# HKUST-Aerial-Robotics/MIND

Hardware: AMD Instinct MI355X
Metric: sim steps/sec (whole node) + scenario-tree nodes expanded/sec, AV2 demo scenes (higher is better)
Workload: dtype f32-class (bf16 hi+mid+lo split operands = 24 significand bits, six products, fp32 accumulate) pair kernel + ActorNet, f32 elsewhere in the predictor, f64 iLQR

## Files before the change

### include/mind_hip.h

```cpp
#ifndef MIND_HIP_H
#define MIND_HIP_H

#include <stddef.h>
#include <stdint.h>

#ifdef __cplusplus
extern "C" {
#endif

#define MIND_OK 0
#define MIND_EINVAL (-1)
#define MIND_ENOMEM (-2)
#define MIND_EHIP (-3)
#define MIND_ESTATE (-4)
#define MIND_ENOTFOUND (-5)

typedef struct mind_ctx mind_ctx;

int mind_ctx_create(int device, void *stream, mind_ctx **out);
int mind_ctx_destroy(mind_ctx *ctx);
const char *mind_last_error_string(mind_ctx *ctx);
int mind_ctx_synchronize(mind_ctx *ctx);

typedef struct {
  const char *name;
  const float *data;
  int64_t numel;
} mind_tensor_desc;

int mind_weights_load(mind_ctx *ctx, const mind_tensor_desc *tensors, int n_tensors);

typedef struct {
  int n_scenes;
  const int32_t *actor_off;
  const int32_t *lane_off;
  const float *actors;
  const float *lanes;
  const float *lane_feat;
  const float *actor_ctrs;
  const float *actor_vecs;
  const float *lane_ctrs;
  const float *lane_vecs;
  const float *const *rpe;
  const float *tgt_nodes;
  const float *tgt_rpe;
} mind_scene_batch;

typedef struct {
  float *cls;
  float *reg;
  float *vel;
  float *lane_feat;
  float *actor_emb;
  float *cls_emb;
} mind_pred_out;

int mind_predict_batch(mind_ctx *ctx, const mind_scene_batch *in, mind_pred_out *out);

typedef struct {
  float *cov_vel;
  float *param;
} mind_pred_aux;
int mind_predict_batch_aux(mind_ctx *ctx, const mind_scene_batch *in, mind_pred_out *out, const mind_pred_aux *aux);

#define MIND_BASIS_BEZIER 0
#define MIND_BASIS_MONOMIAL 1
int mind_set_decoder_basis(mind_ctx *ctx, int basis);
int mind_get_decoder_basis(mind_ctx *ctx);

#define MIND_CURVE_MAX_POINTS (1LL << 26)
int mind_curve_eval(mind_ctx *ctx, int basis, const float *param, long long n_rows, const double *tau, int n_tau,
                    float *reg, float *vel, float *cov_vel);
int mind_debug_curve_basis(int basis, const double *tau, int n_tau, float *T, float *Tp);

int mind_last_fusion_stats(mind_ctx *ctx, int *n_launches, float *total_ms, double *pairs_processed);
int mind_last_actor_stats(mind_ctx *ctx, int *layerwise, int *n_launches, int *n_chunks, float *total_ms);
int mind_last_token_stats(mind_ctx *ctx, int *layerwise, int *n_launches, int *n_chunks, float *total_ms);
int mind_last_token_stage_ms(mind_ctx *ctx, float *out_ms, int cap);
int mind_last_ilqr_stats(mind_ctx *ctx, float *kernel_ms, int *n_trees, int *workgroups_per_tree);
int mind_last_ilqr_profile(mind_ctx *ctx, double *out9);
int mind_last_ilqr_trace(mind_ctx *ctx, int tree, int phase, double *out, int cap_rows, int *n_rows);
int mind_set_profiling(mind_ctx *ctx, int enable);

#define MIND_PAIR_F32 0
#define MIND_PAIR_BF16X3 1
#define MIND_PAIR_BF16 2
#define MIND_PAIR_BF16X6 3
int mind_set_pair_precision(mind_ctx *ctx, int mode);

int mind_set_tuning(mind_ctx *ctx, const char *name, int value);
int mind_get_pair_precision(mind_ctx *ctx);
int mind_debug_pack_bfrag(const float *w, int row_stride, uint32_t *out);

int mind_debug_pair_schedule(const int *scene_tokens, const int *scene_actors, int n_scenes, int n_cu, int last_layer, int *out_jobs, int cap,
                             int *out_info);

int mind_debug_predict_choice(const char *const *knob_names, const int *knob_values, int n_knobs, int pair_prec, int n_cu, int have_side,
                              const int *scene_actors, const int *scene_lanes, int n_scenes, long long *out, int cap);

int mind_debug_ilqr_plan(const char *const *knob_names, const int *knob_values, int n_knobs, int n_cu, int mode, int n_trees, const int *n_nodes,
                         const int32_t *parents, long long *out, int cap, int *bad);

int mind_debug_aime_book(int pred_len, int max_depth, int max_rounds, int n_agents, int world, int rank, int force, int n_rounds, const int *dec_len,
                         const float *dec, int n_tokens, int bytes_per_pair, int plan_chunk_mb, int per_scene, long long *out, int cap, char *msg,
                         int msg_cap);

int mind_debug_wait_word(const unsigned *word, unsigned want, double timeout_s, double (*clock)(void *user), void *user, int spins_per_look);

int mind_debug_actor_lw_plan(int n_actors, int np, int chunk, long long *out_launches, int cap, long long *out_info);

int mind_debug_token_lw_plan(int n_tokens, int mode, int chunk, long long *out_launches, int cap, long long *out_info);

int mind_debug_pack_conv_frag(const float *w, int co, int ci, int ksz, uint32_t *out, size_t cap);

int mind_debug_pack(const char *what, const float *w, int a, int b, int c, float *out, size_t cap);
int mind_debug_weight_image(const mind_tensor_desc *tensors, int n_tensors, float *blob, size_t blob_cap, char *names, size_t names_cap,
                            long long *entries, int entries_cap, long long *out_info, char *msg, int msg_cap);
int mind_debug_weight_bind(const mind_tensor_desc *tensors, int n_tensors, const char *drop, char *msg, int msg_cap);

int mind_debug_trig(mind_ctx *ctx, const double *x, int n, double *out);

int mind_debug_set_layers(mind_ctx *ctx, int n);
int64_t mind_debug_read(mind_ctx *ctx, const char *name, float *host, int64_t max_floats);

typedef struct {
  int n_nodes;
  const int32_t *parent;
  const float *prob;
  int n_agents;
  const float *agent_mean;
  const float *agent_cov;
  const double *field;
  const double *node_w;
} mind_cost_tree;

typedef struct {
  double dt, wheelbase;
  double w_des_state[6];
  double w_state_con[6];
  double state_lower[6], state_upper[6];
  double w_ctrl[2];
  double w_tgt, w_ego, w_ego_cov_offset, w_exo, w_exo_cov_offset, w_exo_cost_offset;
  double grid_res; int grid_w, grid_h;
  int max_iter;
} mind_ilqr_cfg;

typedef struct { int iterations; int converged; double J; double mu; } mind_ilqr_stats;

int mind_ilqr_solve_trees(mind_ctx *ctx, const mind_ilqr_cfg *cfg, const mind_cost_tree *trees,
                          int n_trees, const double *x0, const double *target_lane, int n_lane_pts,
                          double target_vel, int use_exo, const double *us_init, double *xs,
                          double *us, mind_ilqr_stats *stats);

int mind_ilqr_contingency(mind_ctx *ctx, const mind_ilqr_cfg *cfg_warm, const mind_ilqr_cfg *cfg_full,
                          const mind_cost_tree *trees, int n_trees, const double *x0,
                          const double *target_lane, int n_lane_pts, double target_vel, double *xs,
                          double *us, mind_ilqr_stats *stats_warm, mind_ilqr_stats *stats_full);
int mind_ilqr_contingency_begin(mind_ctx *ctx, const mind_ilqr_cfg *cfg_warm, const mind_ilqr_cfg *cfg_full,
                                const mind_cost_tree *trees, int n_trees, const double *x0,
                                const double *target_lane, int n_lane_pts, double target_vel, double *xs,
                                double *us, mind_ilqr_stats *stats_warm, mind_ilqr_stats *stats_full);
int mind_ilqr_contingency_begin_plan(mind_ctx *ctx, const mind_ilqr_cfg *cfg_warm, const mind_ilqr_cfg *cfg_full, const double *x0,
                                     const double *target_lane, int n_lane_pts, double target_vel, double *xs, double *us,
// ... 334 lines not shown
```

### mind_amd/_lib.py

```python
import ctypes as C
import os

_HERE = os.path.dirname(os.path.abspath(__file__))
LIB_PATH = os.environ.get("MIND_HIP_LIB", os.path.join(_HERE, "libmind_hip.so"))

WAIT_CLOCK = C.CFUNCTYPE(C.c_double, C.c_void_p)
MIND_OK = 0
MIND_EINVAL, MIND_ENOMEM, MIND_EHIP, MIND_ESTATE, MIND_ENOTFOUND = -1, -2, -3, -4, -5


class TensorDesc(C.Structure):
    _fields_ = [("name", C.c_char_p), ("data", C.POINTER(C.c_float)), ("numel", C.c_int64)]


class SceneBatch(C.Structure):
    _fields_ = [("n_scenes", C.c_int), ("actor_off", C.POINTER(C.c_int32)), ("lane_off", C.POINTER(C.c_int32)),
                ("actors", C.c_void_p), ("lanes", C.c_void_p), ("lane_feat", C.c_void_p),
                ("actor_ctrs", C.c_void_p), ("actor_vecs", C.c_void_p), ("lane_ctrs", C.c_void_p),
                ("lane_vecs", C.c_void_p), ("rpe", C.POINTER(C.c_void_p)), ("tgt_nodes", C.c_void_p),
                ("tgt_rpe", C.c_void_p)]


class PredOut(C.Structure):
    _fields_ = [("cls", C.c_void_p), ("reg", C.c_void_p), ("vel", C.c_void_p), ("lane_feat", C.c_void_p),
# ... 108 lines not shown

class AimeNode(C.Structure):
    _fields_ = [("round", C.c_int), ("scene", C.c_int), ("mode", C.c_int), ("parent", C.c_int), ("prob", C.c_float),
                ("cur_t", C.c_int), ("end_t", C.c_int), ("flags", C.c_int), ("dur", C.c_int), ("row_off", C.c_int64),
                ("tgt_pts", C.c_float * 22)]


class AimePlanOut(C.Structure):
    _fields_ = [("nodes", C.POINTER(AimeNode)), ("n_nodes", C.c_int), ("rows", C.POINTER(C.c_float)), ("n_row_floats", C.c_int64),
                ("n_expanded", C.c_int), ("n_rounds", C.c_int), ("root_flags", C.c_int), ("round_scenes", C.c_int * 32),
                ("pair_ms", C.c_float), ("pair_launches", C.c_int), ("n_trees", C.c_int), ("tree_top", C.POINTER(C.c_int32)),
                ("tree_off", C.POINTER(C.c_int32)), ("flat_parent", C.POINTER(C.c_int32)), ("flat_prob", C.POINTER(C.c_float)),
                ("flat_mean", C.POINTER(C.c_float)), ("flat_cov", C.POINTER(C.c_float)), ("solves_begun", C.c_int)]


class IlqrCfg(C.Structure):
    _fields_ = [("dt", C.c_double), ("wheelbase", C.c_double), ("w_des_state", C.c_double * 6),
                ("w_state_con", C.c_double * 6), ("state_lower", C.c_double * 6), ("state_upper", C.c_double * 6),
                ("w_ctrl", C.c_double * 2), ("w_tgt", C.c_double), ("w_ego", C.c_double),
                ("w_ego_cov_offset", C.c_double), ("w_exo", C.c_double), ("w_exo_cov_offset", C.c_double),
                ("w_exo_cost_offset", C.c_double), ("grid_res", C.c_double), ("grid_w", C.c_int), ("grid_h", C.c_int),
                ("max_iter", C.c_int)]


class IlqrStats(C.Structure):
    _fields_ = [("iterations", C.c_int), ("converged", C.c_int), ("J", C.c_double), ("mu", C.c_double)]


LOOP_TAN_FN = C.CFUNCTYPE(C.c_double, C.c_double)
LOOP_SINCOS_FN = C.CFUNCTYPE(None, C.c_double, C.POINTER(C.c_double))


class LoopDesc(C.Structure):
    _fields_ = [("n_tracks", C.c_int), ("n_steps", C.c_int), ("clamp_last", C.c_int), ("ego_state", C.c_void_p), ("ego_state_is_f32", C.c_int), ("ego_obs", C.c_void_p), ("ego_trig32", C.c_void_p),
                ("tan_fn", C.c_void_p), ("sincos_fn", C.c_void_p), ("exo_obs", C.c_void_p),
                ("exo_valid", C.c_void_p), ("timestep", C.c_void_p), ("type_slot", C.c_void_p),
                ("sim_step", C.c_double), ("plan_step", C.c_double), ("enable_time", C.c_double),
                ("wheelbase", C.c_double), ("max_speed", C.c_double), ("max_steer", C.c_double), ("max_acc", C.c_double), ("max_dec", C.c_double),
                ("n_lanes", C.c_int), ("lane_pts", C.c_void_p), ("lane_flags", C.c_void_p),
                ("n_lane_pts", C.c_int), ("target_lane", C.c_void_p), ("target_lane_info", C.c_void_p),
                ("time_ahead", C.c_double), ("min_vel", C.c_float), ("dist_thres", C.c_float), ("max_depth", C.c_int), ("max_rounds", C.c_int),
                ("pred_len", C.c_int), ("prob_floor", C.c_float),
                ("cfg_warm", C.c_void_p), ("cfg_full", C.c_void_p), ("solve_n_lane_pts", C.c_int), ("solve_lane", C.c_void_p), ("target_vel", C.c_double),
                ("eval_n_lane_pts", C.c_int), ("eval_lane_is_f32", C.c_int), ("eval_lane", C.c_void_p), ("speculative", C.c_int)]


class LoopTotals(C.Structure):
    _fields_ = [("plans", C.c_longlong), ("expansions", C.c_longlong), ("scen_trees", C.c_longlong), ("rounds", C.c_longlong),
                ("aime_s", C.c_double), ("ilqr_s", C.c_double), ("total_s", C.c_double),
                ("iterations", C.c_longlong), ("node_iterations", C.c_longlong), ("node_iterations_exo", C.c_longlong),
                ("warm_speculated", C.c_longlong), ("warm_hits", C.c_longlong),
                ("pair_ms", C.c_double), ("pair_launches", C.c_longlong), ("scene_n2", C.c_double), ("scene_n_a1", C.c_double),
                ("ilqr_ms", C.c_double), ("ilqr_launches", C.c_longlong), ("ilqr_trees", C.c_longlong), ("ilqr_workgroups_per_tree", C.c_int),
                ("ilqr_prof", C.c_double * 9), ("ilqr_node_steps", C.c_double)]


class LoopOut(C.Structure):
    _fields_ = [("planned", C.c_int), ("enabled", C.c_int), ("n_steps", C.c_longlong), ("n_plans", C.c_longlong), ("episode_steps", C.c_longlong),
                ("sim_time", C.c_double), ("last_trigger", C.c_double), ("state", C.c_double * 4), ("ctrl", C.c_double * 2),
                ("n_agents", C.c_int), ("n_trees", C.c_int), ("best", C.c_int), ("n_expanded", C.c_int), ("n_rounds", C.c_int), ("n_traj_nodes", C.c_int),
                ("costs", C.POINTER(C.c_double)), ("aime_s", C.c_double), ("ilqr_s", C.c_double), ("total_s", C.c_double),
                ("tot", LoopTotals)]


PLANNER_EGO_KEY = -(1 << 63)


class PlannerDesc(C.Structure):
    _fields_ = [("time_ahead", C.c_double), ("min_vel", C.c_float), ("dist_thres", C.c_float), ("max_depth", C.c_int), ("max_rounds", C.c_int),
                ("pred_len", C.c_int), ("prob_floor", C.c_float), ("cfg_warm", C.c_void_p), ("cfg_full", C.c_void_p), ("speculative", C.c_int),
                ("ego_type_slot", C.c_int)]


class PlannerOut(C.Structure):
    _fields_ = [("n_plans", C.c_longlong),
                ("n_agents", C.c_int), ("n_trees", C.c_int), ("best", C.c_int), ("n_expanded", C.c_int), ("n_rounds", C.c_int), ("n_traj_nodes", C.c_int),
                ("costs", C.POINTER(C.c_double)), ("ctrl", C.c_double * 2), ("aime_s", C.c_double), ("ilqr_s", C.c_double), ("total_s", C.c_double),
                ("tot", LoopTotals)]


EXPORTS = ["mind_ctx_create", "mind_ctx_destroy", "mind_last_error_string", "mind_ctx_synchronize",
           "mind_weights_load", "mind_predict_batch", "mind_last_fusion_stats", "mind_last_actor_stats", "mind_debug_actor_lw_plan", "mind_last_token_stats", "mind_last_token_stage_ms", "mind_debug_token_lw_plan", "mind_set_profiling",
           "mind_ilqr_solve_trees", "mind_ilqr_contingency", "mind_ilqr_solve_fields", "mind_cost_eval", "mind_ilqr_score_trees", "mind_ilqr_gains", "mind_ilqr_policy_rollouts", "mind_lane_dist_field", "mind_aime_world", "mind_aime_rebase", "mind_debug_aime_decide", "mind_debug_set_layers",
           "mind_debug_read", "mind_set_pair_precision", "mind_get_pair_precision", "mind_debug_pack_bfrag", "mind_debug_pack_conv_frag", "mind_debug_pack", "mind_debug_weight_image", "mind_debug_weight_bind", "mind_debug_pair_schedule", "mind_debug_predict_choice", "mind_debug_ilqr_plan", "mind_debug_aime_book", "mind_set_tuning", "mind_last_ilqr_stats", "mind_aime_plan", "mind_last_ilqr_profile", "mind_eval_traj_trees", "mind_last_ilqr_trace", "mind_ilqr_contingency_begin", "mind_ilqr_finish", "mind_fill_tracks", "mind_ilqr_contingency_begin_plan", "mind_debug_trig", "mind_aime_plan_begin", "mind_aime_plan_poll", "mind_aime_plan_finish", "mind_ctx_busy", "mind_ilqr_finish_plan",
           "mind_set_exchange", "mind_last_exchange_stats", "mind_debug_wait_word",
           "mind_predict_batch_aux", "mind_set_decoder_basis", "mind_get_decoder_basis", "mind_curve_eval", "mind_debug_curve_basis",
           "mind_audit_plan", "mind_audit_episode", "mind_debug_box_clearance",
           "mind_forecast_score", "mind_debug_forecast_score",
           "mind_audit_road_plan", "mind_audit_road_episode", "mind_debug_road_margin",
           "mind_loop_create", "mind_loop_destroy", "mind_loop_reset", "mind_loop_advance", "mind_loop_state", "mind_loop_last_plan", "mind_loop_export",
           "mind_planner_create", "mind_planner_destroy", "mind_planner_reset", "mind_planner_observe", "mind_planner_set_lanes", "mind_planner_set_target_lane",
           "mind_planner_set_solve_lane", "mind_planner_set_eval_lane", "mind_planner_plan", "mind_planner_last_plan", "mind_planner_export"]

EXCHANGE_FN = C.CFUNCTYPE(C.c_int, C.c_void_p, C.c_int, C.c_void_p, C.c_void_p, C.c_int64)
XCHG_ALLGATHER, XCHG_ALLREDUCE, XCHG_ALLTOALLV = 0, 1, 2

_lib = None


def load():
    global _lib
    if _lib is not None:
        return _lib
    if not os.path.exists(LIB_PATH):
        raise ImportError(f"{LIB_PATH} is missing: the HIP extension must be built (hipcc --offload-arch=gfx950); "
                          "there is no CPU fallback for the product path")
    lib = C.CDLL(LIB_PATH)
    lib.mind_ctx_create.argtypes = [C.c_int, C.c_void_p, C.POINTER(C.c_void_p)]
    lib.mind_ctx_destroy.argtypes = [C.c_void_p]
    lib.mind_last_error_string.argtypes = [C.c_void_p]
    lib.mind_last_error_string.restype = C.c_char_p
    lib.mind_ctx_synchronize.argtypes = [C.c_void_p]
    lib.mind_weights_load.argtypes = [C.c_void_p, C.POINTER(TensorDesc), C.c_int]
    lib.mind_predict_batch.argtypes = [C.c_void_p, C.POINTER(SceneBatch), C.POINTER(PredOut)]
    lib.mind_predict_batch_aux.argtypes = [C.c_void_p, C.POINTER(SceneBatch), C.POINTER(PredOut), C.POINTER(PredAux)]
    lib.mind_set_decoder_basis.argtypes = [C.c_void_p, C.c_int]
    lib.mind_get_decoder_basis.argtypes = [C.c_void_p]
    lib.mind_curve_eval.argtypes = [C.c_void_p, C.c_int, C.c_void_p, C.c_longlong, C.POINTER(C.c_double), C.c_int, C.c_void_p, C.c_void_p, C.c_void_p]
    lib.mind_debug_curve_basis.argtypes = [C.c_int, C.POINTER(C.c_double), C.c_int, C.POINTER(C.c_float), C.POINTER(C.c_float)]
    lib.mind_last_fusion_stats.argtypes = [C.c_void_p, C.POINTER(C.c_int), C.POINTER(C.c_float), C.POINTER(C.c_double)]
    lib.mind_last_actor_stats.argtypes = [C.c_void_p, C.POINTER(C.c_int), C.POINTER(C.c_int), C.POINTER(C.c_int), C.POINTER(C.c_float)]
    lib.mind_debug_actor_lw_plan.argtypes = [C.c_int, C.c_int, C.c_int, C.POINTER(C.c_longlong), C.c_int, C.POINTER(C.c_longlong)]
    lib.mind_last_token_stats.argtypes = [C.c_void_p, C.POINTER(C.c_int), C.POINTER(C.c_int), C.POINTER(C.c_int), C.POINTER(C.c_float)]
    lib.mind_last_token_stage_ms.argtypes = [C.c_void_p, C.POINTER(C.c_float), C.c_int]
    lib.mind_debug_token_lw_plan.argtypes = [C.c_int, C.c_int, C.c_int, C.POINTER(C.c_longlong), C.c_int, C.POINTER(C.c_longlong)]
    lib.mind_set_profiling.argtypes = [C.c_void_p, C.c_int]
    lib.mind_ilqr_solve_trees.argtypes = [C.c_void_p, C.POINTER(IlqrCfg), C.POINTER(CostTree), C.c_int,
                                          C.POINTER(C.c_double), C.POINTER(C.c_double), C.c_int, C.c_double, C.c_int,
                                          C.POINTER(C.c_double), C.POINTER(C.c_double), C.POINTER(C.c_double),
                                          C.POINTER(IlqrStats)]
    lib.mind_ilqr_contingency.argtypes = [C.c_void_p, C.POINTER(IlqrCfg), C.POINTER(IlqrCfg), C.POINTER(CostTree), C.c_int,
                                          C.POINTER(C.c_double), C.POINTER(C.c_double), C.c_int, C.c_double,
                                          C.POINTER(C.c_double), C.POINTER(C.c_double), C.POINTER(IlqrStats), C.POINTER(IlqrStats)]
    lib.mind_ilqr_contingency_begin.argtypes = [C.c_void_p, C.POINTER(IlqrCfg), C.POINTER(IlqrCfg), C.POINTER(CostTree), C.c_int,
                                          C.POINTER(C.c_double), C.POINTER(C.c_double), C.c_int, C.c_double,
                                          C.POINTER(C.c_double), C.POINTER(C.c_double), C.POINTER(IlqrStats), C.POINTER(IlqrStats)]
    lib.mind_ilqr_finish.argtypes = [C.c_void_p]
    lib.mind_ilqr_contingency_begin_plan.argtypes = [C.c_void_p, C.POINTER(IlqrCfg), C.POINTER(IlqrCfg), C.c_void_p, C.c_void_p, C.c_int, C.c_double,
                                                     C.c_void_p, C.c_void_p, C.c_void_p, C.c_void_p]
    lib.mind_fill_tracks.argtypes = [C.c_void_p, C.c_int, C.c_int, C.c_void_p, C.c_void_p, C.c_void_p, C.c_void_p, C.c_void_p, C.c_void_p]
    lib.mind_ilqr_solve_fields.argtypes = [C.c_void_p, C.POINTER(IlqrCfg), C.POINTER(FieldGrid), C.POINTER(CostTree), C.c_int,
                                           C.POINTER(C.c_double), C.POINTER(C.c_double), C.POINTER(C.c_double),
                                           C.POINTER(C.c_double), C.POINTER(IlqrStats)]
    lib.mind_cost_eval.argtypes = [C.c_void_p, C.POINTER(IlqrCfg), C.POINTER(FieldGrid), C.POINTER(CostTree),
                                   C.POINTER(C.c_double), C.POINTER(C.c_double), C.c_int, C.c_double, C.c_int, C.c_int,
                                   C.POINTER(C.c_int32), C.POINTER(C.c_double), C.POINTER(C.c_double), C.POINTER(C.c_double)]
    lib.mind_ilqr_score_trees.argtypes = [C.c_void_p, C.POINTER(IlqrCfg), C.POINTER(FieldGrid), C.POINTER(CostTree), C.c_int,
                                          C.POINTER(C.c_double), C.POINTER(C.c_double), C.c_int, C.c_double, C.c_int, C.c_int,
                                          C.POINTER(C.c_double), C.POINTER(C.c_double), C.POINTER(C.c_double), C.POINTER(C.c_double)]
    lib.mind_ilqr_gains.argtypes = [C.c_void_p, C.POINTER(IlqrCfg), C.POINTER(FieldGrid), C.POINTER(CostTree), C.c_int,
                                    C.POINTER(C.c_double), C.POINTER(C.c_double), C.c_int, C.c_double, C.c_int,
                                    C.POINTER(C.c_double), C.POINTER(C.c_double), C.POINTER(IlqrGainsOut)]
    lib.mind_ilqr_policy_rollouts.argtypes = [C.c_void_p, C.POINTER(IlqrCfg), C.POINTER(FieldGrid), C.POINTER(CostTree), C.c_int,
                                              C.POINTER(C.c_double), C.POINTER(C.c_double), C.c_int, C.c_double, C.c_int,
                                              C.POINTER(C.c_double), C.POINTER(C.c_double), C.POINTER(C.c_double), C.c_int,
                                              C.POINTER(C.c_double), C.POINTER(C.c_double), C.POINTER(C.c_double), C.POINTER(C.c_double),
                                              C.POINTER(C.c_double), C.POINTER(C.c_double)]
    lib.mind_lane_dist_field.argtypes = [C.c_void_p, C.POINTER(C.c_double), C.POINTER(C.c_double), C.c_int, C.c_int, C.c_int,
                                         C.c_double] + [C.POINTER(C.c_double)] * 4
    lib.mind_aime_world.argtypes = [C.c_void_p, C.POINTER(WorldIn), C.POINTER(WorldOut)]
    lib.mind_aime_rebase.argtypes = [C.c_void_p, C.POINTER(RebaseIn), C.POINTER(RebaseOut)]
    lib.mind_debug_aime_decide.argtypes = [C.c_void_p, C.c_int, C.POINTER(C.c_int32), C.POINTER(C.c_int32), C.c_void_p, C.POINTER(C.c_float), C.c_void_p,
                                           C.c_void_p, C.c_void_p, C.c_int, C.c_float, C.c_float, C.c_int, C.c_int, C.c_void_p, C.c_void_p, C.c_void_p]
    lib.mind_aime_plan.argtypes = [C.c_void_p, C.POINTER(AimePlanIn), C.POINTER(AimePlanOut)]
    lib.mind_aime_plan_begin.argtypes = [C.c_void_p, C.POINTER(AimePlanIn)]
    lib.mind_aime_plan_poll.argtypes = [C.c_void_p]
    lib.mind_aime_plan_finish.argtypes = [C.c_void_p, C.POINTER(AimePlanOut)]
    lib.mind_ctx_busy.argtypes = [C.c_void_p]
    lib.mind_ilqr_finish_plan.argtypes = [C.c_void_p, C.c_int, C.c_int, C.c_void_p, C.c_void_p, C.c_void_p, C.c_void_p]
    lib.mind_set_pair_precision.argtypes = [C.c_void_p, C.c_int]
    lib.mind_set_tuning.argtypes = [C.c_void_p, C.c_char_p, C.c_int]
    lib.mind_last_ilqr_stats.argtypes = [C.c_void_p, C.POINTER(C.c_float), C.POINTER(C.c_int), C.POINTER(C.c_int)]
    lib.mind_last_ilqr_profile.argtypes = [C.c_void_p, C.POINTER(C.c_double)]
    lib.mind_last_ilqr_trace.argtypes = [C.c_void_p, C.c_int, C.c_int, C.POINTER(C.c_double), C.c_int, C.POINTER(C.c_int)]
    lib.mind_eval_traj_trees.argtypes = [C.POINTER(C.c_double), C.POINTER(C.c_double), C.POINTER(C.c_int32), C.c_int, C.c_void_p, C.c_int, C.c_int,
                                         C.c_double, C.POINTER(C.c_double)]
    lib.mind_get_pair_precision.argtypes = [C.c_void_p]
    lib.mind_debug_pack_bfrag.argtypes = [C.POINTER(C.c_float), C.c_int, C.POINTER(C.c_uint32)]
    lib.mind_debug_pair_schedule.argtypes = [C.POINTER(C.c_int), C.POINTER(C.c_int), C.c_int, C.c_int, C.c_int, C.POINTER(C.c_int), C.c_int, C.POINTER(C.c_int)]
    lib.mind_debug_predict_choice.argtypes = [C.POINTER(C.c_char_p), C.POINTER(C.c_int), C.c_int, C.c_int, C.c_int, C.c_int, C.POINTER(C.c_int), C.POINTER(C.c_int),
                                              C.c_int, C.POINTER(C.c_longlong), C.c_int]
    lib.mind_debug_ilqr_plan.argtypes = [C.POINTER(C.c_char_p), C.POINTER(C.c_int), C.c_int, C.c_int, C.c_int, C.c_int, C.POINTER(C.c_int), C.POINTER(C.c_int32),
                                         C.POINTER(C.c_longlong), C.c_int, C.POINTER(C.c_int)]
    lib.mind_debug_wait_word.argtypes = [C.POINTER(C.c_uint), C.c_uint, C.c_double, WAIT_CLOCK, C.c_void_p, C.c_int]
    lib.mind_debug_aime_book.argtypes = [C.c_int] * 8 + [C.POINTER(C.c_int), C.POINTER(C.c_float)] + [C.c_int] * 4 + [C.POINTER(C.c_longlong), C.c_int, C.c_char_p, C.c_int]
    lib.mind_debug_trig.argtypes = [C.c_void_p, C.POINTER(C.c_double), C.c_int, C.POINTER(C.c_double)]
    lib.mind_debug_pack_conv_frag.argtypes = [C.POINTER(C.c_float), C.c_int, C.c_int, C.c_int, C.POINTER(C.c_uint32), C.c_size_t]
    lib.mind_debug_pack.argtypes = [C.c_char_p, C.POINTER(C.c_float), C.c_int, C.c_int, C.c_int, C.POINTER(C.c_float), C.c_size_t]
    lib.mind_debug_weight_image.argtypes = [C.POINTER(TensorDesc), C.c_int, C.POINTER(C.c_float), C.c_size_t, C.c_char_p, C.c_size_t,
                                            C.POINTER(C.c_longlong), C.c_int, C.POINTER(C.c_longlong), C.c_char_p, C.c_int]
    lib.mind_debug_weight_bind.argtypes = [C.POINTER(TensorDesc), C.c_int, C.c_char_p, C.c_char_p, C.c_int]
    lib.mind_debug_set_layers.argtypes = [C.c_void_p, C.c_int]
    lib.mind_debug_read.argtypes = [C.c_void_p, C.c_char_p, C.POINTER(C.c_float), C.c_int64]
    lib.mind_set_exchange.argtypes = [C.c_void_p, C.c_int, C.c_int, EXCHANGE_FN, C.c_void_p, C.c_int]
    lib.mind_last_exchange_stats.argtypes = [C.c_void_p, C.POINTER(C.c_longlong), C.POINTER(C.c_longlong)]
    lib.mind_loop_create.argtypes = [C.c_void_p, C.POINTER(LoopDesc), C.POINTER(C.c_void_p)]
    lib.mind_loop_destroy.argtypes = [C.c_void_p]
    lib.mind_loop_reset.argtypes = [C.c_void_p]
    lib.mind_loop_advance.argtypes = [C.c_void_p, C.c_int, C.c_double, C.c_longlong, C.POINTER(LoopOut)]
    lib.mind_loop_state.argtypes = [C.c_void_p, C.POINTER(LoopOut)]
    lib.mind_loop_last_plan.argtypes = [C.c_void_p, C.POINTER(AimePlanOut)] + [C.POINTER(C.c_void_p)] * 6 + [C.c_void_p]
    lib.mind_loop_export.argtypes = [C.c_void_p, C.c_int, C.POINTER(C.c_int), C.c_void_p, C.c_void_p, C.c_void_p]
    lib.mind_planner_create.argtypes = [C.c_void_p, C.POINTER(PlannerDesc), C.POINTER(C.c_void_p)]
    lib.mind_planner_destroy.argtypes = [C.c_void_p]
    lib.mind_planner_reset.argtypes = [C.c_void_p]
    lib.mind_planner_observe.argtypes = [C.c_void_p, C.c_int, C.c_void_p, C.c_int, C.c_void_p, C.c_void_p, C.c_void_p]
    lib.mind_planner_set_lanes.argtypes = [C.c_void_p, C.c_int, C.c_void_p, C.c_void_p]
    lib.mind_planner_set_target_lane.argtypes = [C.c_void_p, C.c_int, C.c_void_p, C.c_void_p]
    lib.mind_planner_set_solve_lane.argtypes = [C.c_void_p, C.c_int, C.c_void_p, C.c_double]
    lib.mind_planner_set_eval_lane.argtypes = [C.c_void_p, C.c_int, C.c_void_p, C.c_int]
    lib.mind_planner_plan.argtypes = [C.c_void_p, C.c_void_p, C.c_void_p, C.POINTER(PlannerOut)]
    lib.mind_planner_last_plan.argtypes = [C.c_void_p, C.POINTER(AimePlanOut)] + [C.POINTER(C.c_void_p)] * 6 + [C.c_void_p]
    lib.mind_planner_export.argtypes = [C.c_void_p, C.c_int, C.POINTER(C.c_int), C.c_void_p, C.c_void_p, C.c_void_p]
    lib.mind_audit_plan.argtypes = [C.c_void_p, C.POINTER(AuditBox), C.c_double, C.POINTER(CostTree), C.c_int, C.c_int, C.POINTER(C.c_double),
                                    C.POINTER(AuditPlanOut)]
    lib.mind_audit_episode.argtypes = [C.c_void_p, C.POINTER(AuditBox), C.c_int, C.c_int, C.c_int, C.POINTER(C.c_double), C.POINTER(C.c_double),
                                       C.POINTER(C.c_uint8), C.POINTER(C.c_double), C.POINTER(AuditEpisodeOut)]
    lib.mind_debug_box_clearance.argtypes = [C.c_int, C.c_int, C.POINTER(C.c_double), C.POINTER(C.c_double), C.POINTER(C.c_double), C.POINTER(C.c_double)]
    fc_tail = [C.POINTER(ForecastCfg), C.c_int, C.POINTER(C.c_int32), C.c_void_p, C.c_void_p, C.POINTER(C.c_double), C.POINTER(C.c_uint8),
               C.POINTER(C.c_uint8), C.POINTER(ForecastOut)]
    lib.mind_forecast_score.argtypes = [C.c_void_p] + fc_tail
    lib.mind_debug_forecast_score.argtypes = fc_tail
    road = [C.POINTER(C.c_double), C.POINTER(C.c_int32), C.c_int]
    lib.mind_audit_road_plan.argtypes = [C.c_void_p, C.POINTER(AuditBox)] + road + [C.POINTER(CostTree), C.c_int, C.c_int, C.POINTER(C.c_double),
                                                                                   C.POINTER(AuditRoadPlanOut)]
    lib.mind_audit_road_episode.argtypes = [C.c_void_p, C.POINTER(AuditBox)] + road + [C.c_int, C.c_int, C.POINTER(C.c_double),
                                                                                      C.POINTER(AuditRoadEpisodeOut)]
    lib.mind_debug_road_margin.argtypes = [C.c_int, C.POINTER(C.c_double), C.POINTER(AuditBox)] + road + [C.POINTER(C.c_double), C.POINTER(C.c_double)] + \
        [C.POINTER(C.c_int32)] * 3
    for n in EXPORTS:
        getattr(lib, n)
        if n not in ("mind_last_error_string", "mind_debug_read"):
            getattr(lib, n).restype = C.c_int
    lib.mind_debug_read.restype = C.c_int64
    _lib = lib
    return lib


PRED_CHOICE_FIELDS = ("header", "n_runs", "np", "actor_form", "actor_arg", "actor_grid", "actor_chunk", "actor_chunks", "actor_launches", "qsplit", "qk_stride",
                      "tiled", "edge_bf16", "edge_pair_bytes", "tok_chunk", "tok_lw", "tok_chunks", "pair_family", "pair_np", "l5_jobs5", "xcd_lanes",
                      "xcd_lanes5", "dec_actor", "dec_np", "fp32_dec", "split_dec", "want_mw", "mw_blocks", "cls_on_side", "tgt_wait_first",
                      "dec_head_ra")
PAIR_PREC = ("f32", "bf16x3", "bf16", "bf16x6")


def predict_choice(knobs, prec, scenes, n_cu=256, have_side=True):
    lib = load()
    names = (C.c_char_p * max(1, len(knobs)))(*[k.encode() for k in knobs])
    vals = (C.c_int * max(1, len(knobs)))(*[int(v) for v in knobs.values()])
    sa = (C.c_int * len(scenes))(*[a for a, _ in scenes])
    sl = (C.c_int * len(scenes))(*[l for _, l in scenes])
    cap = 32 + 6 * len(scenes)
    out = (C.c_longlong * cap)()
    n = lib.mind_debug_predict_choice(names, vals, len(knobs), PAIR_PREC.index(prec) if isinstance(prec, str) else prec, n_cu, int(have_side),
                                      sa, sl, len(scenes), out, cap)
    if n == MIND_EINVAL:
# ... 256 lines not shown
```

### mind_amd/csrc/aime_plan.hip

```cpp
#include <chrono>
namespace {

int pl_pin(mind_ctx *c, int which, size_t bytes) {
  if (bytes <= c->pl_pin_cap[which]) return MIND_OK;
  if (c->pl_pin[which]) (void)hipHostFree(c->pl_pin[which]);
  c->pl_pin[which] = nullptr; c->pl_pin_cap[which] = 0;
  const size_t want = bytes < ((size_t)64 << 20) ? std::max<size_t>(2 * bytes, (size_t)1 << 20) : bytes + bytes / 2 + 4096;
  if (hipHostMalloc(&c->pl_pin[which], want, hipHostMallocDefault) != hipSuccess)
    return fail(c, MIND_ENOMEM, "hipHostMalloc(%zu) failed", want);
  c->pl_pin_cap[which] = want;
  return MIND_OK;
}

struct CopySeg { const float *src; float *dst; long long n; };
__global__ __launch_bounds__(256) void k_copy_segs(const CopySeg *__restrict__ segs) {
  const CopySeg S = segs[blockIdx.y];
  const long long i0 = (long long)blockIdx.x * 2048 + threadIdx.x;
#pragma unroll
  for (int k = 0; k < 8; ++k) {
    const long long i = i0 + k * 256;
    if (i < S.n) S.dst[i] = S.src[i];
  }
}

int pl_exchange(mind_ctx *c, int op, void *send, void *recv, size_t bytes) {
  HIPCHK(c, hipStreamSynchronize(c->stream));
  const int rc = c->xfn(c->xuser, op, send, recv, (int64_t)bytes);
  if (rc) return fail(c, MIND_EHIP, "mind_aime_plan: the exchange callback failed (%d)", rc);
  c->x_collectives += 1;
  c->x_bytes += op == MIND_XCHG_ALLGATHER ? (long long)bytes * c->xw : (long long)bytes;
  return MIND_OK;
}

int pl_exchange_v(mind_ctx *c, void *send, void *recv, const int64_t *table) {
  HIPCHK(c, hipStreamSynchronize(c->stream));
  const int rc = c->xfn(c->xuser, MIND_XCHG_ALLTOALLV, send, recv, (int64_t)(intptr_t)table);
  if (rc) return fail(c, MIND_EHIP, "mind_aime_plan: the exchange callback failed (%d)", rc);
  c->x_collectives += 1;
  for (int r = 0; r < c->xw; ++r) c->x_bytes += (long long)table[(size_t)c->xw + r];
  return MIND_OK;
}

int pl_copy_segs(mind_ctx *c, const std::vector<CopySeg> &segs) {
  if (segs.empty()) return MIND_OK;
  long long mx = 0;
  for (const CopySeg &s : segs) mx = std::max(mx, s.n);
  if (mx == 0) return MIND_OK;
  int rc;
  if ((rc = ensure(c, c->x_seg, segs.size() * sizeof(CopySeg)))) return rc;
  if ((rc = pl_pin(c, 6, segs.size() * sizeof(CopySeg)))) return rc;
  memcpy(c->pl_pin[6], segs.data(), segs.size() * sizeof(CopySeg));
  HIPCHK(c, hipMemcpyAsync(c->x_seg.p, c->pl_pin[6], segs.size() * sizeof(CopySeg), hipMemcpyHostToDevice, c->stream));
  hipLaunchKernelGGL(k_copy_segs, dim3((unsigned)((mx + 2047) / 2048), (unsigned)segs.size()), dim3(256), 0, c->stream, (const CopySeg *)c->x_seg.p);
  HIPCHK(c, hipGetLastError());
  return MIND_OK;
}

static_assert(PL_K == AIME_K && PL_OBS == RB_T, "aime_book.h restates the kernels' constants");
static_assert(sizeof(PlJob) == sizeof(AimeGather) && sizeof(PlJob) == sizeof(AimeFlat) && offsetof(PlJob, row0) == offsetof(AimeGather, row0) &&
                  offsetof(PlJob, row0) == offsetof(AimeFlat, row0) && offsetof(PlJob, n) == offsetof(AimeGather, dur) && offsetof(PlJob, n) == offsetof(AimeFlat, n) &&
                  offsetof(PlJob, dst) == offsetof(AimeGather, dst) && offsetof(PlJob, dst) == offsetof(AimeFlat, dst) && offsetof(PlJob, a) == offsetof(AimeGather, a) &&
                  offsetof(PlJob, a) == offsetof(AimeFlat, a), "JobTable holds the packing kernels' job records");

struct PlTrace {
  std::chrono::steady_clock::time_point t0 = std::chrono::steady_clock::now();
  void operator()(const char *what) const {
    static const bool on = getenv("MIND_PLAN_TRACE") != nullptr;
    if (on) fprintf(stderr, "[plan] %8.1f us  %s\n", std::chrono::duration<double, std::micro>(std::chrono::steady_clock::now() - t0).count(), what);
  }
};

double pl_steady_now(void *) { return std::chrono::duration<double>(std::chrono::steady_clock::now().time_since_epoch()).count(); }

struct PlanRun {
  mind_ctx *c;
  const mind_aime_plan_in *in;
  mind_aime_plan_out *out;
  hipStream_t st;
  AimeBook &book;
  const int a, l, P, HZ;
  const bool raw;
  const int XW, XR;
  const bool dist;
  const RootLayout ro;
  const float *droot = nullptr;
  int cur_in = -1;
  const float *prev_pos = nullptr, *prev_ang = nullptr, *prev_vel = nullptr, *cov_last_dev = nullptr;
// ... 428 lines not shown
    if (n_hdr && XR == 0) segs.push_back({(const float *)c->pl_lf.p, snd, (long long)n_hdr});
    if (r.Sm > 0) segs.push_back({fr_base + (size_t)r.s0 * 28, snd + n_hdr, (long long)r.Sm * 28});
    if ((rc = pl_copy_segs(c, segs))) return rc;
    if ((rc = pl_exchange(c, MIND_XCHG_ALLGATHER, snd, rcv, n_pay * sizeof(float)))) return rc;
    segs.clear();
    if (n_hdr && XR != 0) segs.push_back({rcv, (float *)c->pl_lf.p, (long long)n_hdr});
    for (int k = 0; k < XW; ++k) {
      if (k == XR || r.cnt_r[k] == 0) continue;
      segs.push_back({rcv + (size_t)k * n_pay + n_hdr, fr_base + (size_t)r.s0_r[k] * 28, (long long)r.cnt_r[k] * 28});
    }
    if ((rc = pl_copy_segs(c, segs))) return rc;
  }
  size_t per_scene = 0;
  for (int k = 0; k < 11; ++k) per_scene += arrs[k].per;
  PlRoute rt;
  pl_route(r.S, XW, XR, r.cnt_r, r.s0_r, per_scene, c->xforce != 0, rt);
  if (rt.any <= 0) return MIND_OK;
  size_t n_snd = 0, n_rcv = 0;
  for (int k = 0; k < XW; ++k) { n_snd += (size_t)rt.tab[k] / sizeof(float); n_rcv += (size_t)rt.tab[(size_t)XW + k] / sizeof(float); }
  if ((rc = ensure(c, c->x_send, (n_snd + 4) * sizeof(float)))) return rc;
  if ((rc = ensure(c, c->x_recv, (n_rcv + 4) * sizeof(float)))) return rc;
  float *snd = (float *)c->x_send.p, *rcv = (float *)c->x_recv.p;
  const auto pair_segs = [&](const std::vector<int> &range, float *packed, bool unpack) {
    segs.clear();
    size_t o = 0;
    for (int k = 0; k < XW; ++k) {
      const size_t i0 = range[2 * k], n = range[2 * k + 1] - range[2 * k];
      for (int e = 0; e < 11 && n > 0; ++e) {
        float *arr = arrs[e].base + arrs[e].per * i0;
        segs.push_back(unpack ? CopySeg{packed + o, arr, (long long)(arrs[e].per * n)} : CopySeg{arr, packed + o, (long long)(arrs[e].per * n)});
        o += arrs[e].per * n;
      }
    }
  };
  pair_segs(rt.snd, snd, false);
  if ((rc = pl_copy_segs(c, segs))) return rc;
  if ((rc = pl_exchange_v(c, snd, rcv, rt.tab.data()))) return rc;
  pair_segs(rt.rcv, rcv, true);
  return pl_copy_segs(c, segs);
}

int PlanRun::pl_next_inputs() {
  const int S = book.rec.S;
  int nlo, nhi, rc;
  pl_block(S, XR, XW, nlo, nhi);
  const int n_rep = nhi - nlo;
  if (n_rep > 1 && (rc = ensure(c, c->pl_lrep, (size_t)n_rep * l * 128 * sizeof(float)))) return rc;
  const auto rep = [this, n_rep](hipStream_t rs) {
    if (n_rep > 1) {
      const size_t n = (size_t)l * 128;
      hipLaunchKernelGGL(k_repeat_rows, dim3((unsigned)((n * n_rep + 255) / 256)), dim3(256), 0, rs, (const float *)c->pl_lf.p, n, n_rep, (float *)c->pl_lrep.p);
      HIPCHK(c, hipGetLastError());
    }
    return (int)MIND_OK;
  };
  const float *d_fr = d_in + q.fr;
  const auto back = [this, d_fr, S](hipStream_t rs) { return pl_frames_back(d_fr, (size_t)S, rs); };
  if (c->round_head && c->side && !dist) {
    c->enc_pre = rep; c->enc_post = back;
  } else {
    hipStream_t rs;
    if ((rc = pl_side_hop(rs)) || (rc = rep(rs)) || (rc = back(rs))) return rc;
  }
  prev_pos = w_pos; prev_ang = w_ang; prev_vel = w_vel;
  cov_last_dev = d_in + q.cov;
  cur_in = nxt;
  return MIND_OK;
}

void PlanRun::pl_begin_solves() {
  const size_t Mtot = (size_t)book.tree_off.back(), nt = book.tree_top.size();
  c->pl_sol_xs.resize(Mtot * 6); c->pl_sol_us.resize(Mtot * 2);
  c->pl_sol_stw.resize(nt); c->pl_sol_stf.resize(nt);
  solves_tried = true;
  solves_rc = mind_ilqr_contingency_begin_plan(c, in->solve_cfg_warm, in->solve_cfg_full, in->solve_x0, in->solve_lane, in->solve_n_lane_pts,
                                               in->solve_target_vel, c->pl_sol_xs.data(), c->pl_sol_us.data(), c->pl_sol_stw.data(), c->pl_sol_stf.data());
  c->il_finish_owned = solves_rc == MIND_OK;
}

int PlanRun::pl_pack_results() {
  const size_t Mtot = (size_t)book.tree_off.back(), n_rows = (size_t)book.n_rows, n_flat = Mtot * a * 3, n_res = n_rows + n_flat;
  want_solves = solves_asked() && !book.tree_top.empty();
  int rc;
  c->plan.agents = a;
  c->plan.rows_p = c->plan.fmean_p = c->plan.fcov_p = nullptr;
  c->plan.dev_fmean = c->plan.dev_fcov = nullptr;
  if (n_res > 0) {
    const JobTable &F = book.flat, &G = book.gather;
    const size_t o_g = F.bytes(), n_tab = o_g + G.bytes();
    const size_t o_rows = (n_tab + 255) & ~(size_t)255;
    if ((rc = ensure(c, c->pl_flat, o_rows + n_res * sizeof(float)))) return rc;
    if ((rc = pl_pin(c, 0, n_tab))) return rc;
    char *h = (char *)c->pl_pin[0];
    const float *world_of_round[32];
    for (size_t i = 0; i < c->pl_world.size() && i < 32; ++i) world_of_round[i] = (const float *)c->pl_world[i].p;
    F.pack(h, world_of_round);
    G.pack(h + o_g, world_of_round);
    TR("end: trees flattened on the host");
    const bool tab_host = !dist && c->tab_host_max > 0 && F.job_of_block.size() + G.job_of_block.size() <= (size_t)c->tab_host_max;
    if (n_tab && !tab_host) HIPCHK(c, hipMemcpyAsync(c->pl_flat.p, h, n_tab, hipMemcpyHostToDevice, st));
    char *d = tab_host ? h : (char *)c->pl_flat.p;
    float *d_rows = (float *)((char *)c->pl_flat.p + o_rows), *d_fmean = d_rows + n_rows, *d_fcov = d_fmean + Mtot * a * 2;
    if (dist) HIPCHK(c, hipMemsetAsync(d_rows, 0, n_res * sizeof(float), st));
    if (!F.jobs.empty())
      hipLaunchKernelGGL(k_aime_flat, dim3((unsigned)F.job_of_block.size()), dim3(64), 0, st, (const AimeFlat *)d, (const int *)(d + F.off_job()),
                         (const int *)(d + F.off_agent()), (const float *const *)(d + F.off_world()), d_fmean, d_fcov);
    const auto gather = [&](hipStream_t gs) {
      if (!G.jobs.empty())
        hipLaunchKernelGGL(k_aime_gather, dim3((unsigned)G.job_of_block.size()), dim3(64), 0, gs, (const AimeGather *)(d + o_g), (const int *)(d + o_g + G.off_job()),
                           (const int *)(d + o_g + G.off_agent()), (const float *const *)(d + o_g + G.off_world()), d_rows);
    };
    if (!want_solves) gather(st);
    HIPCHK(c, hipGetLastError());
    if (dist && (rc = pl_exchange(c, MIND_XCHG_ALLREDUCE, d_rows, d_rows, n_res * sizeof(float)))) return rc;
    c->plan.dev_fmean = d_fmean; c->plan.dev_fcov = d_fcov;
    if ((rc = pl_pin(c, 2, n_res * sizeof(float)))) return rc;
    float *hp = (float *)c->pl_pin[2];
    if (want_solves) {
      if (!c->ev_rows) HIPCHK(c, hipEventCreateWithFlags(&c->ev_rows, hipEventDisableTiming));
      HIPCHK(c, hipEventRecord(c->ev_tab, st));
      TR("end: flat kernel queued");
      pl_begin_solves();
      TR("end: solves begun");
      HIPCHK(c, hipStreamWaitEvent(c->pl_copy, c->ev_tab, 0));
      gather(c->pl_copy);
      HIPCHK(c, hipGetLastError());
      HIPCHK(c, hipMemcpyAsync(hp, d_rows, n_res * sizeof(float), hipMemcpyDeviceToHost, c->pl_copy));
      HIPCHK(c, hipEventRecord(c->ev_rows, c->pl_copy));
      HIPCHK(c, hipEventSynchronize(c->ev_rows));
      TR("end: read-back on the host");
    } else {
      HIPCHK(c, hipMemcpyAsync(hp, d_rows, n_res * sizeof(float), hipMemcpyDeviceToHost, st));
      HIPCHK(c, hipStreamSynchronize(st));
    }
    c->plan.rows_p = hp; c->plan.fmean_p = hp + n_rows; c->plan.fcov_p = hp + n_rows + Mtot * a * 2;
  } else {
    HIPCHK(c, hipStreamSynchronize(st));
  }
  return MIND_OK;
}

int PlanRun::pl_hand_out() {
  float pair_ms = 0.f;
  int rc;
  out->nodes = book.table.data(); out->n_nodes = (int)book.table.size();
  out->rows = c->plan.rows_p; out->n_row_floats = book.n_rows;
  out->n_expanded = n_expanded; out->n_rounds = book.n_rounds;
  out->root_flags = book.root_flags();
  if (c->profiling && (rc = mind_pair_events_resolve(c, &pair_ms))) return rc;
  out->pair_ms = pair_ms; out->pair_launches = pair_launches;
  out->n_trees = (int)book.tree_top.size(); out->tree_top = book.tree_top.data(); out->tree_off = book.tree_off.data();
  out->flat_parent = book.flat_parent.data(); out->flat_prob = book.flat_prob.data();
  out->flat_mean = c->plan.fmean_p; out->flat_cov = c->plan.fcov_p;
  if (want_solves) {
    if (!solves_tried) pl_begin_solves();
    out->solves_begun = solves_rc == MIND_OK ? 1 : 0;
  }
  TR("end: result handed out");
  return MIND_OK;
}

}

extern "C" int mind_aime_plan(mind_ctx *c, const mind_aime_plan_in *in, mind_aime_plan_out *out) {
  if (!c || !in || !out) return MIND_EINVAL;
  int rc;
// ... 149 lines not shown
```

### mind_amd/csrc/ilqr_host.hip

```cpp
static void il_make_grid(int W, int H, double res, const double *ego_xy, double *gx, double *gy, double &offx, double &offy) {
  const double fsx = (double)(W - 1) * res, fsy = (double)(H - 1) * res;
  offx = ego_xy[0] - 0.5 * fsx; offy = ego_xy[1] - 0.5 * fsy;
  const double sx = fsx / (double)(W - 1), sy = fsy / (double)(H - 1);
  for (int i = 0; i < W; ++i) gx[i] = (double)i * sx + 0.0;
  gx[W - 1] = fsx;
  for (int i = 0; i < H; ++i) gy[i] = (double)i * sy + 0.0;
  gy[H - 1] = fsy;
  for (int i = 0; i < W; ++i) gx[i] += offx;
  for (int i = 0; i < H; ++i) gy[i] += offy;
}

extern "C" int mind_lane_dist_field(mind_ctx *c, const double *ego_xy, const double *lane, int n_pts, int W, int H,
                                    double res, double *offset, double *gx, double *gy, double *dist) {
  if (!c || !ego_xy || !lane || n_pts < 2 || W < 2 || H < 2 || !(res > 0) || !offset || !gx || !gy || !dist)
    return fail(c, MIND_EINVAL, "mind_lane_dist_field: bad argument");
  HIPCHK(c, hipSetDevice(c->device));
  hipStream_t st = c->stream;
  il_make_grid(W, H, res, ego_xy, gx, gy, offset[0], offset[1]);
  const size_t nd = (size_t)W + H + 2 * (size_t)n_pts + (size_t)W * H;
  int rc;
  if ((rc = ensure(c, c->ilqr_dev, nd * sizeof(double)))) return rc;
  double *d = (double *)c->ilqr_dev.p;
  HIPCHK(c, hipMemcpyAsync(d, gx, W * sizeof(double), hipMemcpyHostToDevice, st));
  HIPCHK(c, hipMemcpyAsync(d + W, gy, H * sizeof(double), hipMemcpyHostToDevice, st));
  HIPCHK(c, hipMemcpyAsync(d + W + H, lane, 2 * (size_t)n_pts * sizeof(double), hipMemcpyHostToDevice, st));
  double *out = d + W + H + 2 * (size_t)n_pts;
  hipLaunchKernelGGL(k_lane_field, dim3((W * H + 255) / 256), dim3(256), 0, st, d, d + W, W, H, d + W + H, n_pts, out, 0);
  HIPCHK(c, hipGetLastError());
  HIPCHK(c, hipMemcpyAsync(dist, out, (size_t)W * H * sizeof(double), hipMemcpyDeviceToHost, st));
  HIPCHK(c, hipStreamSynchronize(st));
  return MIND_OK;
}

namespace { int pl_pin(mind_ctx *c, int which, size_t bytes); }

typedef unsigned up_u4 __attribute__((ext_vector_type(4)));
__global__ __launch_bounds__(256) void k_upload(const up_u4 *__restrict__ src, up_u4 *__restrict__ dst, size_t n16) {
  for (size_t i = (size_t)blockIdx.x * 256 + threadIdx.x; i < n16; i += (size_t)gridDim.x * 256) dst[i] = __builtin_nontemporal_load(src + i);
}
static int pl_upload(mind_ctx *c, void *dst, const void *pinned_src, size_t bytes, hipStream_t s) {
  if (!bytes) return MIND_OK;
  if (c->upload_kernel_max > 0 && bytes <= (size_t)c->upload_kernel_max && bytes % 16 == 0 && (uintptr_t)dst % 16 == 0 && (uintptr_t)pinned_src % 16 == 0) {
    const size_t n16 = bytes / 16;
    hipLaunchKernelGGL(k_upload, dim3((unsigned)std::min<size_t>((n16 + 255) / 256, 256)), dim3(256), 0, s, (const up_u4 *)pinned_src, (up_u4 *)dst, n16);
    HIPCHK(c, hipGetLastError());
    return MIND_OK;
  }
  HIPCHK(c, hipMemcpyAsync(dst, pinned_src, bytes, hipMemcpyHostToDevice, s));
  return MIND_OK;
}

static int il_field_prepare(mind_ctx *c, const mind_ilqr_cfg *cfg, const double *x0, const double *lane, int n_lane_pts, hipStream_t s) {
  c->il_field_valid = false;
  const int W = cfg->grid_w, H = cfg->grid_h;
  if (W < 3 || H < 3 || n_lane_pts < 2 || !(cfg->grid_res > 0)) return MIND_OK;
  const size_t nin = (size_t)W + H + 2 * (size_t)n_lane_pts, nd = nin + (size_t)W * H;
  int rc;
  if ((rc = ensure(c, c->il_field, nd * sizeof(double)))) return rc;
  if (c->il_field_pin_cap < nin * sizeof(double)) {
    if (c->il_field_pin) (void)hipHostFree(c->il_field_pin);
    c->il_field_pin = nullptr; c->il_field_pin_cap = 0;
    if (hipHostMalloc(&c->il_field_pin, 2 * nin * sizeof(double), hipHostMallocDefault) != hipSuccess) { c->il_field_pin = nullptr; return MIND_OK; }
    c->il_field_pin_cap = 2 * nin * sizeof(double);
  }
  if (!c->ev_field) HIPCHK(c, hipEventCreateWithFlags(&c->ev_field, hipEventDisableTiming));
  double *h = (double *)c->il_field_pin, ox, oy;
  il_make_grid(W, H, cfg->grid_res, x0, h, h + W, ox, oy);
  memcpy(h + W + H, lane, 2 * (size_t)n_lane_pts * sizeof(double));
  double *d = (double *)c->il_field.p;
  HIPCHK(c, hipMemcpyAsync(d, h, nin * sizeof(double), hipMemcpyHostToDevice, s));
  hipLaunchKernelGGL(k_lane_field, dim3((W * H + 255) / 256), dim3(256), 0, s, d, d + W, W, H, d + W + H, n_lane_pts, d + nin);
  HIPCHK(c, hipGetLastError());
  HIPCHK(c, hipEventRecord(c->ev_field, s));
  c->il_field_key[0] = x0[0]; c->il_field_key[1] = x0[1]; c->il_field_key[2] = W; c->il_field_key[3] = H; c->il_field_key[4] = cfg->grid_res;
  c->il_field_lane.assign(lane, lane + 2 * (size_t)n_lane_pts);
  c->il_field_valid = true;
  return MIND_OK;
}

struct IlqrEvalReq { int nq; const int32_t *node; const double *x, *u; double *out; };
struct IlqrScoreReq { int n_cand; const double *us_cand; double *xs, *L, *J; };
#define IL_SCORE_MAX_ROWS (1L << 20)
struct IlqrGainsReq { const double *us, *mu; const mind_ilqr_gains_out *out; };
struct IlqrPolicyReq { int n_cand; const double *us, *k, *K, *alpha, *dx0; double *xs, *us_out, *L, *J; };

struct IlqrCall {
  const mind_ilqr_cfg *cfg = nullptr, *cfg2 = nullptr;
  const mind_field_grid *grid = nullptr;
  const mind_cost_tree *trees = nullptr;
  int n_trees = 0;
  const double *x0 = nullptr, *lane = nullptr;
  int n_lane_pts = 0;
  double target_vel = 0.0;
  int use_exo = 0;
  const double *us_init = nullptr;
  double *xs = nullptr, *us = nullptr;
  mind_ilqr_stats *stats = nullptr, *stats2 = nullptr;
  const IlqrEvalReq *ev = nullptr;
  const IlqrScoreReq *sc = nullptr;
  const IlqrGainsReq *ga = nullptr;
  const IlqrPolicyReq *po = nullptr;
  bool begin_only = false;
  bool dev_flat = false;
};

struct IlRun {
  const IlqrCall &q;
  bool gen = false, dev_flat = false, field_ahead = false;
  int n_phases = 1, use_exo = 0, use_exo_first = 0, n_lane_pts = 0, W = 0, H = 0, trace_cap = 0, amax = 1;
  int pol_cb = 0;
  long Mtot = 0;
  double grid_res = 0, fsx = 0, fsy = 0, offx = 0, offy = 0;
  std::vector<double> gx, gy;
  std::vector<int> n_agents;
  IlqrChoice ch;
  IlArena A;
  char *base = nullptr;
  const char *up = nullptr;
  double *hx = nullptr, *hus = nullptr;
  unsigned *h_abort = nullptr, *h_done = nullptr;
  size_t n_xs = 0, n_hx = 0, n_us = 0;
  std::vector<IlqrTreeDev> hT;
  IlqrConst K[2];
  explicit IlRun(const IlqrCall &call) : q(call) {}
  double *Dp(size_t o) const { return o < A.nd_in ? (double *)base + o : (double *)(base + A.o_work) + (o - A.nd_in); }
  float *dF() const { return (float *)(base + A.bytesIn); }
  int *dI() const { return (int *)(base + A.bytesIn + A.bytesF); }
};

struct IlStamp {
  const std::chrono::steady_clock::time_point t0 = std::chrono::steady_clock::now();
  void operator()(const char *what) const {
    static const bool on = getenv("MIND_PLAN_TRACE") != nullptr;
    if (on) fprintf(stderr, "[ilqr] %8.1f us  %s\n", std::chrono::duration<double, std::micro>(std::chrono::steady_clock::now() - t0).count(), what);
  }
};

static int il_check(mind_ctx *c, const IlqrCall &q, IlRun &R) {
  const mind_ilqr_cfg *cfg = q.cfg, *cfg2 = q.cfg2;
  const IlqrEvalReq *ev = q.ev;
// ... 182 lines not shown
    IlqrTreeDev &D = R.hT[t];
    D.M = tr.n_nodes; D.n_agents = (int)a; D.n_levels = T.nl; D.pad = 0;
    D.parent = dI + L.parent; D.level_start = dI + L.lstart; D.level_nodes = dI + L.lnodes;
    D.child_start = dI + L.cstart; D.child_list = dI + L.clist;
    D.rel = dI + L.rel;
    D.relag = R.Dp(L.relag);
    D.field = gen ? (const double *)(R.base + L.field) : nullptr;
    D.node_w = gen ? R.Dp(L.nodew) : nullptr;
    D.n_segs = T.nseg; D.n_slevels = T.nsl; D.max_level_segs = T.maxls; D.pad2 = 0;
    D.seg_start = dI + L.sstart; D.seg_nodes = dI + L.snodes; D.slevel_start = dI + L.slstart; D.slevel_segs = dI + L.slsegs; D.seg_rec = dI + L.segrec;
    D.n_fsteps = T.nfs; D.padf = 0;
    D.trace = R.trace_cap > 0 ? R.Dp(L.trace) : nullptr; D.trace_cap = R.trace_cap; D.padt = 0;
    D.fstep_start = dI + L.fsstart; D.fstep_q0 = dI + L.fsitems; D.fstep_q1 = dI + L.fsq1; D.fstep_nstart = dI + L.fsnstart; D.fstep_nodes = dI + L.fsnodes;
    D.prob = dF + L.prob; D.mean = dF + L.mean; D.cov = dF + L.cov;
    if (R.dev_flat) { D.mean = c->plan.dev_fmean + (size_t)moff * a * 2; D.cov = c->plan.dev_fcov + (size_t)moff * a; }
    D.xs = R.Dp(L.xs); D.us = R.Dp(L.us); D.Fx = R.Dp(L.Fx); D.L = R.Dp(L.L); D.Lx = R.Dp(L.Lx); D.Lxx = R.Dp(L.Lxx);
    D.k = R.Dp(L.k); D.K = R.Dp(L.K); D.Vx = R.Dp(L.Vx); D.Vxx = R.Dp(L.Vxx);
    D.xs_new = R.Dp(L.xsn); D.us_new = R.Dp(L.usn); D.L_new = R.Dp(L.Ln); D.stats = R.Dp(L.stats);
    D.ctl = ch.form == 2 ? (IlSlotCtl *)(dI + A.o_ctl + A.ctl_ints * (size_t)t) : nullptr;
    D.h_xs = ch.host_out ? R.hx + (L.xs - L0.xs) : nullptr; D.h_us = ch.host_out ? R.hus + (L.us - L0.us) : nullptr;
    D.h_stats = ch.host_out ? R.hx + (L.stats - L0.xs) : nullptr;
    D.h_done = ch.early ? R.h_done + t : nullptr; D.h_gen = c->il_gen; D.pad_h = 0;
    if (ch.early && ((L.xs - L0.xs) != (size_t)moff * 6 || (L.us - L0.us) != (size_t)moff * 2)) return fail(c, MIND_EINVAL, "tree-iLQR arena: results are not contiguous");
    D.dset = ch.spec ? (long long)L.Fx2 - (long long)L.Fx : 0; D.drel = ch.spec ? (long long)L.rel2 - (long long)L.rel : 0;
    if (ch.spec && (L.L2 - L.L != L.Fx2 - L.Fx || L.Lx2 - L.Lx != L.Fx2 - L.Fx || L.Lxx2 - L.Lxx != L.Fx2 - L.Fx || (R.use_exo && L.relag2 - L.relag != L.Fx2 - L.Fx)))
      return fail(c, MIND_EINVAL, "tree-iLQR arena: the two derivative sets are laid out differently");
    moff += (long)M;
  }
  R.field_ahead = !gen && !ev && !q.sc && !q.ga && !q.po && c->il_field_valid && c->il_field_key[0] == q.x0[0] && c->il_field_key[1] == q.x0[1] && c->il_field_key[2] == (double)R.W &&
                  c->il_field_key[3] == (double)R.H && c->il_field_key[4] == R.grid_res && c->il_field_lane.size() == 2 * (size_t)R.n_lane_pts &&
                  memcmp(c->il_field_lane.data(), q.lane, c->il_field_lane.size() * sizeof(double)) == 0;
  c->il_field_valid = false;
  double *quad = R.field_ahead ? (double *)c->il_field.p + (size_t)R.W + R.H + 2 * (size_t)R.n_lane_pts : R.Dp(A.o_quad);
  il_fill_const(R.K[0], q.cfg, R.use_exo_first, R, quad);
  if (q.cfg2) il_fill_const(R.K[1], q.cfg2, 1, R, quad);
  else R.K[1] = R.K[0];
  {
    const auto off = [&R](size_t o) { return (size_t)((const char *)R.Dp(o) - R.base); };
    c->il_dbg[0] = off(L0.L); c->il_dbg[1] = off(L0.Lx); c->il_dbg[2] = off(L0.Lxx); c->il_dbg[3] = off(L0.Fx); c->il_dbg[4] = off(L0.xs);
    c->il_dbg[5] = (size_t)q.trees[0].n_nodes;
  }
  return MIND_OK;
}

static int il_upload(mind_ctx *c, IlRun &R, hipStream_t st) {
  const IlArena &A = R.A;
  const int n_trees = R.q.n_trees;
  for (int t = 0; t < n_trees && R.gen; ++t)
    HIPCHK(c, hipMemcpyAsync(R.base + A.tree[t].field, R.q.trees[t].field, (size_t)R.q.trees[t].n_nodes * R.W * R.H * sizeof(double), hipMemcpyHostToDevice, st));
  int rc;
  if ((rc = pl_pin(c, 4, A.o_work))) return rc;
  char *up = (char *)c->pl_pin[4];
  memset(up, 0, A.o_work);
  memcpy(up, c->il_img.hD.data(), A.bytesIn);
  if (A.bytesF) memcpy(up + A.bytesIn, c->il_img.hF.data(), A.bytesF);
  if (A.bytesI) memcpy(up + A.bytesIn + A.bytesF, c->il_img.hI.data(), A.bytesI);
  if (R.ch.starve_followers) ((unsigned *)(up + A.bytesIn + A.bytesF))[A.o_bars + 4 * (size_t)n_trees + 1] = 1u;
  memcpy(up + A.o_structs, R.hT.data(), (size_t)n_trees * sizeof(IlqrTreeDev));
  memcpy(up + A.o_consts, R.K, 2 * sizeof(IlqrConst));
  R.up = up;
  return pl_upload(c, R.base, up, A.o_work, st);
}

struct IlPending {
  hipStream_t st;
  bool gen;
  int n_trees, n_phases, use_exo, trace_cap;
  long Mtot;
  IlqrChoice ch;
  const IlqrTreeDev *dT;
  const IlqrConst *dK;
  unsigned *dBars;
  size_t il_lds, o_work;
  char *base;
  const char *up;
  const double *d_xs, *d_us;
  double *hx, *hus;
  const unsigned *h_abort;
  size_t n_xs, n_hx, n_us;
  double *xs, *us;
  mind_ilqr_stats *stats, *stats2;
  struct Tree { int M, nl, nseg, nsl, maxls, a; const double *trace; };
  std::vector<Tree> tree;
};

static void il_launch_kernel(const IlPending &P, int form) {
  const IlqrChoice &ch = P.ch;
  const int nt = P.n_trees;
  const dim3 block(IL_THREADS);
  if (P.gen) hipLaunchKernelGGL((k_ilqr<true, 0>), dim3(nt), block, P.il_lds, P.st, P.dT, P.dK, P.n_phases, nt, 1, P.dBars, 0);
  else if (form == 2) hipLaunchKernelGGL((k_ilqr<false, 2>), dim3(ch.grid), block, P.il_lds, P.st, P.dT, P.dK, P.n_phases, nt, ch.GS, P.dBars, ch.spec);
  else if (form == 1) hipLaunchKernelGGL((k_ilqr<false, 1>), dim3(ch.grid), block, P.il_lds, P.st, P.dT, P.dK, P.n_phases, nt, ch.G, P.dBars, 0);
  else hipLaunchKernelGGL((k_ilqr<false, 0>), dim3(nt), block, P.il_lds, P.st, P.dT, P.dK, P.n_phases, nt, 1, P.dBars, 0);
}

static int il_read_back(mind_ctx *c, const IlPending &P) {
  if (P.ch.host_out) return MIND_OK;
  HIPCHK(c, hipMemcpyAsync(P.hx, P.d_xs, P.n_hx * sizeof(double), hipMemcpyDeviceToHost, P.st));
  HIPCHK(c, hipMemcpyAsync(P.hus, P.d_us, P.n_us * sizeof(double), hipMemcpyDeviceToHost, P.st));
  return MIND_OK;
}

static int il_finish_run(mind_ctx *c, const IlPending &P) {
  static const bool trace = getenv("MIND_ILQR_TRACE") != nullptr;
  const int n_trees = P.n_trees, n_phases = P.n_phases;
  int rc;
  HIPCHK(c, hipStreamSynchronize(P.st));
  if (c->profiling) HIPCHK(c, hipEventElapsedTime(&c->ilqr_ms, c->ev_il0, c->ev_il1));
  if (P.ch.form == 1 && *P.h_abort) {
    c->n_ilqr_fallbacks++;
    HIPCHK(c, hipMemcpyAsync(P.base, P.up, P.o_work, hipMemcpyHostToDevice, P.st));
    il_launch_kernel(P, 0);
    HIPCHK(c, hipGetLastError());
    c->ilqr_multi = 1;
    if ((rc = il_read_back(c, P))) return rc;
    HIPCHK(c, hipStreamSynchronize(P.st));
  }
  memcpy(P.xs, P.hx, (size_t)P.Mtot * 6 * sizeof(double));
  memcpy(P.us, P.hus, P.n_us * sizeof(double));
  const auto hstat = [&P](int t, int ph) { return P.hx + P.n_xs + (size_t)2 * IL_NSTAT * t + (size_t)ph * IL_NSTAT; };
  c->il_trace_dev.assign(n_trees, nullptr);
  c->il_trace_its.assign((size_t)2 * n_trees, 0);
  c->il_trace_cap = P.trace_cap; c->il_trace_phases = n_phases;
  for (int t = 0; t < n_trees; ++t) {
    c->il_trace_dev[t] = P.trace_cap > 0 ? P.tree[t].trace : nullptr;
    for (int ph = 0; ph < n_phases; ++ph) c->il_trace_its[2 * t + ph] = (int)hstat(t, ph)[0];
  }
  c->il_spec_req = 0; c->il_spec_hit = 0;
#ifndef IL_PROFILE
  for (int t = 0; t < n_trees; ++t)
    for (int ph = 0; ph < n_phases; ++ph) { c->il_spec_req += (long long)hstat(t, ph)[9]; c->il_spec_hit += (long long)hstat(t, ph)[10]; }
#endif
  double best = -1.0;
  for (int t = 0; t < n_trees; ++t) {
    double tot = 0.0, ph_c[5] = {0, 0, 0, 0, 0}, passes = 0.0;
    for (int ph = 0; ph < n_phases; ++ph) {
      const double *h = hstat(t, ph);
      ph_c[0] += h[4]; ph_c[1] += h[5]; ph_c[2] += h[8]; ph_c[3] += h[6]; ph_c[4] += h[7];
      passes += h[IL_NSTAT - 1];
    }
    for (double v : ph_c) tot += v;
    if (tot > best) {
      best = tot;
      double *o = c->il_prof;
      o[0] = P.tree[t].M; o[1] = P.tree[t].nl; o[2] = passes;
      for (int k = 0; k < 5; ++k) o[3 + k] = ph_c[k];
      o[8] = (double)n_trees;
    }
  }
  for (int ph = 0; ph < n_phases; ++ph) {
    mind_ilqr_stats *so = ph == 0 ? P.stats : P.stats2;
    if (!so) continue;
    for (int t = 0; t < n_trees; ++t) {
      const double *h = hstat(t, ph);
      const IlPending::Tree &T = P.tree[t];
      so[t].iterations = (int)h[0]; so[t].converged = (int)h[1];
      so[t].J = h[2]; so[t].mu = h[3];
      if (!trace) continue;
      fprintf(stderr, "[k_ilqr] tree %d exo %d M %d segs %d seg-levels %d widest %d agents %d it %d passes %.0f: cycles derivatives %.0f backward %.0f state chain %.0f cost pass %.0f select %.0f\n", t,
              n_phases == 2 ? ph : P.use_exo, T.M, T.nseg, T.nsl, T.maxls, T.a, so[t].iterations, h[IL_NSTAT - 1], h[4], h[5], h[8], h[6], h[7]);
#ifdef IL_PROFILE
      fprintf(stderr, "[k_ilqr prof] wave0: chain node (n=%.0f): stage %.0f u+dyn+store %.0f | cost chunk (n=%.0f): stage+loads %.0f field %.0f cost+store %.0f | riccati node (n=%.0f): products %.0f Qxx %.0f solve %.0f update %.0f | deriv block (n=%.0f): setup %.0f tasks %.0f assemble %.0f\n",
              h[13], h[8] / fmax(h[13], 1), h[9] / fmax(h[13], 1),
              h[23], h[10] / fmax(h[23], 1), h[11] / fmax(h[23], 1), h[12] / fmax(h[23], 1),
              h[18], h[14] / fmax(h[18], 1), h[15] / fmax(h[18], 1), h[16] / fmax(h[18], 1), h[17] / fmax(h[18], 1),
              h[22], h[19] / fmax(h[22], 1), h[20] / fmax(h[22], 1), h[21] / fmax(h[22], 1));
#endif
    }
  }
  return MIND_OK;
}

static int il_eval(mind_ctx *c, const IlRun &R, hipStream_t st) {
  const IlqrEvalReq *ev = R.q.ev;
  const IlArena &A = R.A;
  const IlqrTreeDev *dT = (const IlqrTreeDev *)(R.base + A.o_structs);
  const size_t lds = (IL_SCR + (size_t)4 * R.amax) * sizeof(double);
  if (R.gen) hipLaunchKernelGGL(k_cost_eval<true>, dim3(ev->nq), dim3(64), lds, st, dT, R.K[0], ev->nq, R.dI() + A.o_evn, R.Dp(A.o_evx), R.Dp(A.o_evu), R.Dp(A.o_evo));
  else hipLaunchKernelGGL(k_cost_eval<false>, dim3(ev->nq), dim3(64), lds, st, dT, R.K[0], ev->nq, R.dI() + A.o_evn, R.Dp(A.o_evx), R.Dp(A.o_evu), R.Dp(A.o_evo));
  HIPCHK(c, hipGetLastError());
  HIPCHK(c, hipMemcpyAsync(ev->out, R.Dp(A.o_evo), (size_t)ev->nq * IL_EVAL_OUT * sizeof(double), hipMemcpyDeviceToHost, st));
  HIPCHK(c, hipStreamSynchronize(st));
  return MIND_OK;
}

static int il_score(mind_ctx *c, const IlRun &R, hipStream_t st) {
  const IlqrScoreReq *sc = R.q.sc;
  const IlArena &A = R.A;
  const int n_trees = R.q.n_trees;
  const IlqrTreeDev *dT = (const IlqrTreeDev *)(R.base + A.o_structs);
  const int cb = il_score_block(c->it, c->n_cu, n_trees, sc->n_cand);
// ... 3 lines not shown
  if (R.gen) hipLaunchKernelGGL(k_ilqr_score<true>, grid, block, lds, st, dT, R.K[0], n_trees, sc->n_cand, cb, R.Mtot, il_ag_doubles(R.amax), R.Dp(A.o_scu), R.Dp(A.o_scx), R.Dp(A.o_scl), R.Dp(A.o_scj));
  else hipLaunchKernelGGL(k_ilqr_score<false>, grid, block, lds, st, dT, R.K[0], n_trees, sc->n_cand, cb, R.Mtot, il_ag_doubles(R.amax), R.Dp(A.o_scu), R.Dp(A.o_scx), R.Dp(A.o_scl), R.Dp(A.o_scj));
  HIPCHK(c, hipGetLastError());
  if (sc->xs) HIPCHK(c, hipMemcpyAsync(sc->xs, R.Dp(A.o_scx), rows * 6 * sizeof(double), hipMemcpyDeviceToHost, st));
  if (sc->L) HIPCHK(c, hipMemcpyAsync(sc->L, R.Dp(A.o_scl), rows * sizeof(double), hipMemcpyDeviceToHost, st));
  HIPCHK(c, hipMemcpyAsync(sc->J, R.Dp(A.o_scj), (size_t)sc->n_cand * n_trees * sizeof(double), hipMemcpyDeviceToHost, st));
  HIPCHK(c, hipStreamSynchronize(st));
  return MIND_OK;
}

static int il_gains(mind_ctx *c, const IlRun &R, hipStream_t st) {
  const mind_ilqr_gains_out *o = R.q.ga->out;
  const IlArena &A = R.A;
  const int n_trees = R.q.n_trees;
  const IlqrTreeDev *dT = (const IlqrTreeDev *)(R.base + A.o_structs);
  const size_t lds = il_gains_lds_bytes(R.amax), M = (size_t)R.Mtot;
  if (R.gen) hipLaunchKernelGGL(k_ilqr_gains<true>, dim3(n_trees), dim3(IL_PG_THREADS), lds, st, dT, R.K[0], n_trees, il_ag_doubles(R.amax), R.Dp(A.o_gmu), R.Dp(A.o_gk), R.Dp(A.o_gK), R.Dp(A.o_gdv), R.Dp(A.o_gvx), R.Dp(A.o_gvxx), R.Dp(A.o_gxs), R.Dp(A.o_gl), R.Dp(A.o_gj), R.Dp(A.o_gbad));
  else hipLaunchKernelGGL(k_ilqr_gains<false>, dim3(n_trees), dim3(IL_PG_THREADS), lds, st, dT, R.K[0], n_trees, il_ag_doubles(R.amax), R.Dp(A.o_gmu), R.Dp(A.o_gk), R.Dp(A.o_gK), R.Dp(A.o_gdv), R.Dp(A.o_gvx), R.Dp(A.o_gvxx), R.Dp(A.o_gxs), R.Dp(A.o_gl), R.Dp(A.o_gj), R.Dp(A.o_gbad));
  HIPCHK(c, hipGetLastError());
  const size_t span = A.o_gbad + (size_t)n_trees - A.o_gk;
  int rc;
  if ((rc = pl_pin(c, 5, span * sizeof(double)))) return rc;
  const double *h = (const double *)c->pl_pin[5];
  HIPCHK(c, hipMemcpyAsync(c->pl_pin[5], R.Dp(A.o_gk), span * sizeof(double), hipMemcpyDeviceToHost, st));
  HIPCHK(c, hipStreamSynchronize(st));
  const struct { double *dst; size_t src, n; } outs[8] = {{o->k, A.o_gk, 2 * M}, {o->K, A.o_gK, 12 * M}, {o->dV, A.o_gdv, M}, {o->V_x, A.o_gvx, 6 * M},
                                                          {o->V_xx, A.o_gvxx, 36 * M}, {o->xs, A.o_gxs, 6 * M}, {o->L, A.o_gl, M}, {o->J, A.o_gj, (size_t)n_trees}};
  for (const auto &e : outs)
    if (e.dst) memcpy(e.dst, h + (e.src - A.o_gk), e.n * sizeof(double));
  for (int t = 0; t < n_trees; ++t) o->bad_node[t] = (int32_t)h[A.o_gbad - A.o_gk + t];
  return MIND_OK;
}

static int il_policy(mind_ctx *c, const IlRun &R, hipStream_t st, int cb) {
  const IlqrPolicyReq *po = R.q.po;
  const IlArena &A = R.A;
  const int n_trees = R.q.n_trees;
  const IlqrTreeDev *dT = (const IlqrTreeDev *)(R.base + A.o_structs);
  const dim3 grid((po->n_cand + cb - 1) / cb, n_trees), block(IL_SC_THREADS);
  const size_t lds = il_score_lds_bytes(R.amax);
  const size_t rows = (size_t)po->n_cand * (size_t)R.Mtot;
  if (R.gen) hipLaunchKernelGGL(k_ilqr_policy<true>, grid, block, lds, st, dT, R.K[0], n_trees, po->n_cand, cb, R.Mtot, il_ag_doubles(R.amax), R.Dp(A.o_pk), R.Dp(A.o_pK), R.Dp(A.o_pal), R.Dp(A.o_pdx), R.Dp(A.o_pxn), R.Dp(A.o_pxs), R.Dp(A.o_pus), R.Dp(A.o_pl), R.Dp(A.o_pj));
  else hipLaunchKernelGGL(k_ilqr_policy<false>, grid, block, lds, st, dT, R.K[0], n_trees, po->n_cand, cb, R.Mtot, il_ag_doubles(R.amax), R.Dp(A.o_pk), R.Dp(A.o_pK), R.Dp(A.o_pal), R.Dp(A.o_pdx), R.Dp(A.o_pxn), R.Dp(A.o_pxs), R.Dp(A.o_pus), R.Dp(A.o_pl), R.Dp(A.o_pj));
  HIPCHK(c, hipGetLastError());
  if (po->xs) HIPCHK(c, hipMemcpyAsync(po->xs, R.Dp(A.o_pxs), rows * 6 * sizeof(double), hipMemcpyDeviceToHost, st));
  if (po->us_out) HIPCHK(c, hipMemcpyAsync(po->us_out, R.Dp(A.o_pus), rows * 2 * sizeof(double), hipMemcpyDeviceToHost, st));
  if (po->L) HIPCHK(c, hipMemcpyAsync(po->L, R.Dp(A.o_pl), rows * sizeof(double), hipMemcpyDeviceToHost, st));
  HIPCHK(c, hipMemcpyAsync(po->J, R.Dp(A.o_pj), (size_t)po->n_cand * n_trees * sizeof(double), hipMemcpyDeviceToHost, st));
  HIPCHK(c, hipStreamSynchronize(st));
  return MIND_OK;
}

static int il_launch(mind_ctx *c, const IlRun &R, hipStream_t st, IlPending &P) {
  const IlqrCall &q = R.q;
  const IlArena &A = R.A;
  const IlqrChoice &ch = R.ch;
  const int n_trees = q.n_trees;
  if (R.field_ahead) HIPCHK(c, hipStreamWaitEvent(st, c->ev_field, 0));
  else if (!R.gen) hipLaunchKernelGGL(k_lane_field, dim3((R.W * R.H + 255) / 256), dim3(256), 0, st, R.K[0].gx.p, R.K[0].gy.p, R.W, R.H, R.Dp(A.o_lane), R.n_lane_pts, R.Dp(A.o_quad));
  if (q.ev) return il_eval(c, R, st);
  if (q.sc) return il_score(c, R, st);
  if (q.ga) return il_gains(c, R, st);
  if (q.po) return il_policy(c, R, st, R.pol_cb);
  P.st = st; P.gen = R.gen; P.n_trees = n_trees; P.n_phases = R.n_phases; P.use_exo = R.use_exo; P.trace_cap = R.trace_cap; P.Mtot = R.Mtot; P.ch = ch;
  P.dT = (const IlqrTreeDev *)(R.base + A.o_structs); P.dK = (const IlqrConst *)(R.base + A.o_consts);
  P.dBars = (unsigned *)(R.dI() + A.o_bars);
  P.il_lds = il_lds_bytes(R.amax); P.o_work = A.o_work; P.base = R.base; P.up = R.up;
  P.d_xs = R.Dp(A.tree[0].xs); P.d_us = R.Dp(A.tree[0].us);
  P.hx = R.hx; P.hus = R.hus; P.h_abort = R.h_abort; P.n_xs = R.n_xs; P.n_hx = R.n_hx; P.n_us = R.n_us;
  P.xs = q.xs; P.us = q.us; P.stats = q.stats; P.stats2 = q.stats2;
  P.tree.resize(n_trees);
  for (int t = 0; t < n_trees; ++t) {
    const IlTables &T = c->il_tab[t];
    P.tree[t] = {q.trees[t].n_nodes, T.nl, T.nseg, T.nsl, T.maxls, R.n_agents[t], R.Dp(A.tree[t].trace)};
  }
  if (c->profiling) {
    if (!c->ev_il0) { HIPCHK(c, hipEventCreate(&c->ev_il0)); HIPCHK(c, hipEventCreate(&c->ev_il1)); }
    HIPCHK(c, hipEventRecord(c->ev_il0, st));
  }
  c->ilqr_trees = n_trees; c->ilqr_multi = ch.wgs_per_tree; c->ilqr_ms = 0.f;
  il_launch_kernel(P, ch.form);
  HIPCHK(c, hipGetLastError());
  if (c->profiling) HIPCHK(c, hipEventRecord(c->ev_il1, st));
  int rc;
  if ((rc = il_read_back(c, P))) return rc;
  if (ch.form == 1) HIPCHK(c, hipMemcpyAsync(R.h_abort, P.dBars + 4 * (size_t)n_trees, sizeof(unsigned), hipMemcpyDeviceToHost, st));
  return MIND_OK;
}

static int il_solve(mind_ctx *c, const IlqrCall &q) {
  IlRun R(q);
  int rc;
  if ((rc = il_check(c, q, R))) return rc;
  HIPCHK(c, hipSetDevice(c->device));
  hipStream_t st = c->stream;
  IlStamp stamp;
  il_grid(R);
  int maxM = 0;
  for (int t = 0; t < q.n_trees; ++t) maxM = std::max(maxM, q.trees[t].n_nodes);
  const bool other = q.ev || q.sc || q.ga || q.po;
  R.ch = il_choose(c->it, c->n_cu, q.n_trees, maxM, R.Mtot, R.gen, other);
  if ((rc = il_build_tables(c, q))) return rc;
  IlShape shape{R.W, R.H, R.n_lane_pts, q.ev ? q.ev->nq : 0, q.n_trees, R.n_agents.data(), R.gen, R.use_exo != 0, R.dev_flat, R.trace_cap, q.sc ? q.sc->n_cand : 0};
  shape.gains = q.ga != nullptr;
  if (q.po) {
    R.pol_cb = il_score_block(c->it, c->n_cu, q.n_trees, q.po->n_cand);
    shape.n_pol = q.po->n_cand; shape.n_pol_blk = (q.po->n_cand + R.pol_cb - 1) / R.pol_cb;
  }
  il_layout(shape, R.ch, c->il_tab.data(), R.A);
  stamp("tables built");
  if ((rc = il_stage(c, R))) return rc;
  stamp("staged in vectors");
  if ((rc = il_upload(c, R, st))) return rc;
  stamp("upload queued");
  IlPending P;
  if ((rc = il_launch(c, R, st, P)) || other) return rc;
  stamp("kernel launched");
  if (!q.begin_only) return il_finish_run(c, P);
  c->il_finish = [c, P = std::move(P)]() { return il_finish_run(c, P); };
  return MIND_OK;
}

static IlqrCall il_contingency_call(const mind_ilqr_cfg *cfg_warm, const mind_ilqr_cfg *cfg_full, const mind_cost_tree *trees, int n_trees, const double *x0,
                                    const double *target_lane, int n_lane_pts, double target_vel, double *xs, double *us, mind_ilqr_stats *stats_warm,
                                    mind_ilqr_stats *stats_full) {
  IlqrCall q;
  q.cfg = cfg_warm; q.cfg2 = cfg_full; q.trees = trees; q.n_trees = n_trees; q.x0 = x0; q.lane = target_lane; q.n_lane_pts = n_lane_pts;
  q.target_vel = target_vel; q.xs = xs; q.us = us; q.stats = stats_warm; q.stats2 = stats_full;
  return q;
}

extern "C" int mind_ilqr_contingency_begin(mind_ctx *c, const mind_ilqr_cfg *cfg_warm, const mind_ilqr_cfg *cfg_full,
                                           const mind_cost_tree *trees, int n_trees, const double *x0, const double *target_lane,
                                           int n_lane_pts, double target_vel, double *xs, double *us,
                                           mind_ilqr_stats *stats_warm, mind_ilqr_stats *stats_full) {
  if (!c || !cfg_full) return fail(c, MIND_EINVAL, "mind_ilqr_contingency_begin: null configuration");
  IlqrCall q = il_contingency_call(cfg_warm, cfg_full, trees, n_trees, x0, target_lane, n_lane_pts, target_vel, xs, us, stats_warm, stats_full);
  q.begin_only = true;
  return il_solve(c, q);
}

extern "C" int mind_ilqr_contingency_begin_plan(mind_ctx *c, const mind_ilqr_cfg *cfg_warm, const mind_ilqr_cfg *cfg_full, const double *x0,
                                                const double *target_lane, int n_lane_pts, double target_vel, double *xs, double *us,
                                                mind_ilqr_stats *stats_warm, mind_ilqr_stats *stats_full) {
  if (!c || !cfg_full) return fail(c, MIND_EINVAL, "mind_ilqr_contingency_begin_plan: null configuration");
  const int nt = (int)c->plan.book.tree_top.size();
  if (nt <= 0 || c->plan.agents <= 0) return fail(c, MIND_ESTATE, "mind_ilqr_contingency_begin_plan: the context holds no planned cost trees");
  const int a = c->plan.agents;
  std::vector<mind_cost_tree> trees(nt);
  for (int t = 0; t < nt; ++t) {
    const size_t lo = (size_t)c->plan.book.tree_off[t];
    mind_cost_tree &T = trees[t];
    memset(&T, 0, sizeof(T));
    T.n_nodes = c->plan.book.tree_off[t + 1] - c->plan.book.tree_off[t];
    T.parent = c->plan.book.flat_parent.data() + lo; T.prob = c->plan.book.flat_prob.data() + lo;
    T.n_agents = a;
    T.agent_mean = c->plan.fmean_p ? c->plan.fmean_p + lo * a * 2 : nullptr; T.agent_cov = c->plan.fcov_p ? c->plan.fcov_p + lo * a : nullptr;
  }
  IlqrCall q = il_contingency_call(cfg_warm, cfg_full, trees.data(), nt, x0, target_lane, n_lane_pts, target_vel, xs, us, stats_warm, stats_full);
  q.begin_only = true;
  q.dev_flat = true;
  return il_solve(c, q);
}

extern "C" int mind_ilqr_finish(mind_ctx *c) {
  if (!c) return MIND_EINVAL;
  if (!c->il_finish) return fail(c, MIND_ESTATE, "mind_ilqr_finish: no tree-iLQR call was begun on this context");
  std::function<int()> fin = std::move(c->il_finish);
  c->il_finish = nullptr;
  c->il_finish_owned = false;
  c->il_early = mind_ctx::IlEarly();
  return fin();
}

extern "C" int mind_ilqr_contingency(mind_ctx *c, const mind_ilqr_cfg *cfg_warm, const mind_ilqr_cfg *cfg_full,
                                     const mind_cost_tree *trees, int n_trees, const double *x0, const double *target_lane,
                                     int n_lane_pts, double target_vel, double *xs, double *us,
                                     mind_ilqr_stats *stats_warm, mind_ilqr_stats *stats_full) {
  if (!cfg_full) return fail(c, MIND_EINVAL, "mind_ilqr_contingency: null configuration");
  return il_solve(c, il_contingency_call(cfg_warm, cfg_full, trees, n_trees, x0, target_lane, n_lane_pts, target_vel, xs, us, stats_warm, stats_full));
}

extern "C" int mind_ilqr_solve_trees(mind_ctx *c, const mind_ilqr_cfg *cfg, const mind_cost_tree *trees, int n_trees,
                                     const double *x0, const double *target_lane, int n_lane_pts, double target_vel,
                                     int use_exo, const double *us_init, double *xs, double *us,
                                     mind_ilqr_stats *stats) {
  IlqrCall q;
  q.cfg = cfg; q.trees = trees; q.n_trees = n_trees; q.x0 = x0; q.lane = target_lane; q.n_lane_pts = n_lane_pts; q.target_vel = target_vel;
  q.use_exo = use_exo; q.us_init = us_init; q.xs = xs; q.us = us; q.stats = stats;
  return il_solve(c, q);
}

extern "C" int mind_ilqr_solve_fields(mind_ctx *c, const mind_ilqr_cfg *cfg, const mind_field_grid *grid,
                                      const mind_cost_tree *trees, int n_trees, const double *x0,
                                      const double *us_init, double *xs, double *us, mind_ilqr_stats *stats) {
  if (!grid) return fail(c, MIND_EINVAL, "mind_ilqr_solve_fields: null grid");
  IlqrCall q;
  q.cfg = cfg; q.grid = grid; q.trees = trees; q.n_trees = n_trees; q.x0 = x0; q.us_init = us_init; q.xs = xs; q.us = us; q.stats = stats;
  return il_solve(c, q);
}

extern "C" int mind_cost_eval(mind_ctx *c, const mind_ilqr_cfg *cfg, const mind_field_grid *grid, const mind_cost_tree *tree,
                              const double *x0, const double *target_lane, int n_lane_pts, double target_vel, int use_exo,
                              int n_query, const int32_t *node, const double *x, const double *u, double *out) {
  if (n_query <= 0 || !node || !x || !u || !out) return fail(c, MIND_EINVAL, "mind_cost_eval: bad argument");
  const IlqrEvalReq ev{n_query, node, x, u, out};
  IlqrCall q;
  q.cfg = cfg; q.grid = grid; q.trees = tree; q.n_trees = 1; q.x0 = x0; q.lane = target_lane; q.n_lane_pts = n_lane_pts; q.target_vel = target_vel;
  q.use_exo = use_exo; q.ev = &ev;
  return il_solve(c, q);
}

extern "C" int mind_ilqr_score_trees(mind_ctx *c, const mind_ilqr_cfg *cfg, const mind_field_grid *grid, const mind_cost_tree *trees, int n_trees,
                                     const double *x0, const double *target_lane, int n_lane_pts, double target_vel, int use_exo, int n_cand,
                                     const double *us_cand, double *xs, double *L, double *J) {
  const IlqrScoreReq sc{n_cand, us_cand, xs, L, J};
  IlqrCall q;
  q.cfg = cfg; q.grid = grid; q.trees = trees; q.n_trees = n_trees; q.x0 = x0; q.lane = target_lane; q.n_lane_pts = n_lane_pts; q.target_vel = target_vel;
  q.use_exo = use_exo; q.sc = &sc;
  return il_solve(c, q);
}

extern "C" int mind_ilqr_gains(mind_ctx *c, const mind_ilqr_cfg *cfg, const mind_field_grid *grid, const mind_cost_tree *trees, int n_trees,
                               const double *x0, const double *target_lane, int n_lane_pts, double target_vel, int use_exo, const double *us,
                               const double *mu, const mind_ilqr_gains_out *out) {
  const IlqrGainsReq ga{us, mu, out};
  IlqrCall q;
  q.cfg = cfg; q.grid = grid; q.trees = trees; q.n_trees = n_trees; q.x0 = x0; q.lane = target_lane; q.n_lane_pts = n_lane_pts; q.target_vel = target_vel;
  q.use_exo = use_exo; q.us_init = us; q.ga = &ga;
  return il_solve(c, q);
}

extern "C" int mind_ilqr_policy_rollouts(mind_ctx *c, const mind_ilqr_cfg *cfg, const mind_field_grid *grid, const mind_cost_tree *trees, int n_trees,
                                         const double *x0, const double *target_lane, int n_lane_pts, double target_vel, int use_exo,
                                         const double *us, const double *k, const double *K, int n_cand, const double *alpha, const double *dx0,
                                         double *xs, double *us_out, double *L, double *J) {
  const IlqrPolicyReq po{n_cand, us, k, K, alpha, dx0, xs, us_out, L, J};
  IlqrCall q;
  q.cfg = cfg; q.grid = grid; q.trees = trees; q.n_trees = n_trees; q.x0 = x0; q.lane = target_lane; q.n_lane_pts = n_lane_pts; q.target_vel = target_vel;
  q.use_exo = use_exo; q.us_init = us; q.po = &po;
  return il_solve(c, q);
}

#define IL_PLAN_HEADER 16
extern "C" int mind_debug_ilqr_plan(const char *const *knob_names, const int *knob_values, int n_knobs, int n_cu, int mode, int n_trees,
                                    const int *n_nodes, const int32_t *parents, long long *out, int cap, int *bad) {
  if (bad) bad[0] = bad[1] = -1;
  if (n_knobs < 0 || (n_knobs > 0 && (!knob_names || !knob_values)) || n_cu <= 0 || mode < 0 || mode > 7 || n_trees <= 0 || !n_nodes || !parents ||
      cap < 0 || (cap > 0 && !out))
    return MIND_EINVAL;
  IlqrTuning t;
  for (int k = 0; k < n_knobs; ++k)
    if (!knob_names[k] || !ilqr_tuning_set(t, knob_names[k], knob_values[k])) return MIND_EINVAL;
  int maxM = 0;
  long Mtot = 0;
// ... 25 lines not shown
```

### mind_amd/csrc/loop.hip

```cpp
#pragma once
#pragma STDC FP_CONTRACT OFF
#include <chrono>
#include <unordered_map>

namespace {

constexpr int LOOP_OBS = 50;
constexpr int LOOP_ROW = 7;

struct LoopTrack {
  int track = 0;
  long long key = 0;
  int slot = 6;
  int count = 0, head = 0;
  double rows[LOOP_OBS][LOOP_ROW];
  const double *last() const { return rows[(head + count - 1) % LOOP_OBS]; }
  void push(const double *r) {
    double *dst;
    if (count < LOOP_OBS) dst = rows[(head + count++) % LOOP_OBS];
    else { dst = rows[head]; head = (head + 1) % LOOP_OBS; }
    memcpy(dst, r, LOOP_ROW * sizeof(double));
  }
  void push_observed(const double *v, double timestep) {
    double row[LOOP_ROW];
// ... 20 lines not shown
  std::vector<int32_t> lane_flags;
  std::vector<float> target_lane, target_lane_info, eval_lane_f32;
  mind_ilqr_cfg cfg_warm, cfg_full;
  double state[4] = {0, 0, 0, 0}, ctrl[2] = {0, 0};
  std::vector<LoopTrack> obs;
  std::vector<double> raw, eval_st, eval_ct, costs, per;
  std::vector<char> early_seen;
  std::vector<float> f_pos, f_ang, f_vel, f_pad, f_types;
  std::vector<int16_t> i_typ, i_have;
  std::vector<int32_t> kept, kept_obs, slots, counts;
  std::vector<long long> kept_keys;
  mind_aime_plan_out po;
  bool have_plan = false;
  long long plan_gen = -1;
  std::chrono::steady_clock::time_point t_plan_end;
  mind_ctx *side = nullptr;
  hipStream_t side_stream = nullptr;
  struct Shape { std::vector<int32_t> parent; std::vector<float> prob; };
  std::vector<Shape> last_shapes, spec_shapes;
  bool spec_pending = false;
  int spec_skip = 0, spec_backoff = 4, spec_last = -1;
  std::vector<double> spec_xs, spec_us, sol_xs, sol_us, hit_ui, miss_xs, miss_us;
  std::vector<mind_ilqr_stats> spec_st, sol_stw, sol_stf, miss_stw, miss_stf;
  std::vector<float> zero_mean, zero_cov;
  long long warm_speculated = 0, warm_hits = 0;
  double plan_x0[6];
  int last_agents = 0, last_nodes = 0, best = -1, last_agents_plan = 0;
  bool sol_owned = false;
  double aime_s = 0, ilqr_s = 0, total_s = 0;
  mind_loop_totals tot;
  mind_cycle() { memset(&po, 0, sizeof(po)); memset(&tot, 0, sizeof(tot)); }
  int add_track(int track, long long key, int slot) {
    obs.emplace_back();
    obs.back().track = track; obs.back().key = key; obs.back().slot = slot;
    return (int)obs.size() - 1;
  }
};

struct mind_loop : mind_cycle {
  mind_loop_desc d;
  std::vector<double> ego_state, ego_obs, exo_obs;
  std::vector<uint8_t> exo_valid;
  std::vector<int32_t> timestep, type_slot;
  std::vector<float> ego_trig32;
  double sim_time = 0.0, last_trigger = -1.0;
  bool have_trigger = false, enabled = false;
  bool state_recorded = false;
  int state_row = 0;
  bool tan_valid = false;
  double tan_arg = 0.0, tan_val = 0.0;
  long long n_steps = 0, n_plans = 0, ep_steps = 0;
  std::vector<int> slot_of_track;
  bool half_step = false;
  bool planned_last = false;
};

struct mind_planner : mind_cycle {
  std::unordered_map<long long, int> slot_of_key;
  std::vector<long long> frame_keys;
  std::vector<char> frame_seen;
  bool have_lanes = false, have_target = false, have_solve = false, have_eval = false;
  long long n_plans = 0, n_uploads = 0;
};

namespace {

template <class Desc> void cycle_params_from(CycleParams &cp, const Desc &d) {
  cp.time_ahead = d.time_ahead; cp.min_vel = d.min_vel; cp.dist_thres = d.dist_thres; cp.max_depth = d.max_depth; cp.max_rounds = d.max_rounds;
  cp.pred_len = d.pred_len; cp.prob_floor = d.prob_floor; cp.speculative = d.speculative;
}

template <class Out> void cycle_fill_plan_out(const mind_cycle *L, Out *o) {
  if (L->have_plan) {
    o->n_agents = L->last_agents; o->n_trees = L->po.n_trees; o->best = L->best;
    o->n_expanded = L->po.n_expanded; o->n_rounds = L->po.n_rounds;
    o->n_traj_nodes = L->last_nodes;
    o->costs = L->costs.data();
    o->aime_s = L->aime_s; o->ilqr_s = L->ilqr_s; o->total_s = L->total_s;
  }
  o->tot = L->tot;
}

void cycle_drop_speculation(mind_cycle *L) {
  if (L->spec_pending && L->side) { (void)mind_ilqr_finish(L->side); L->spec_pending = false; }
}

template <class Seen> void cycle_repeat_unseen(mind_cycle *L, size_t known_before, Seen seen) {
  double row[LOOP_ROW];
  for (size_t s = 1; s < known_before; ++s) {
    LoopTrack &t = L->obs[s];
    if (seen(s, t)) continue;
    memcpy(row, t.last(), sizeof(row));
    row[0] = 0.0;
    t.push(row);
  }
}

template <class Id> int cycle_last_plan(mind_cycle *L, const std::vector<Id> &idents, mind_aime_plan_out *plan, const double **xs, const double **us,
                                        const mind_ilqr_stats **stats_warm, const mind_ilqr_stats **stats_full, const Id **agents, const float **types, double *x0) {
  if (!L->have_plan) return fail(L->c, MIND_ESTATE, "%s_last_plan: no plan is held", L->who);
  if (L->plan_gen != L->c->plan.gen) return fail(L->c, MIND_ESTATE, "%s_last_plan: the context has planned again since (another planner shares it): the plan's tables are gone", L->who);
  *plan = L->po;
  if (xs) *xs = L->sol_owned ? L->sol_xs.data() : L->c->pl_sol_xs.data();
  if (us) *us = L->sol_owned ? L->sol_us.data() : L->c->pl_sol_us.data();
  if (stats_warm) *stats_warm = L->sol_owned ? L->sol_stw.data() : L->c->pl_sol_stw.data();
  if (stats_full) *stats_full = L->sol_owned ? L->sol_stf.data() : L->c->pl_sol_stf.data();
  if (agents) *agents = idents.data();
  if (types) *types = L->f_types.data();
  if (x0) memcpy(x0, L->plan_x0, 6 * sizeof(double));
  return MIND_OK;
}

template <class M, class Id> void cycle_export_rows(const mind_cycle *L, int first, int n, M LoopTrack::*id, Id *ident, int32_t *count, double *rows) {
  for (int s = 0; s < n; ++s) {
    const LoopTrack &t = L->obs[s + first];
    ident[s] = t.*id; count[s] = t.count;
    for (int k = 0; k < t.count; ++k)
      memcpy(rows + ((size_t)s * LOOP_OBS + k) * LOOP_ROW, t.rows[(t.head + k) % LOOP_OBS], LOOP_ROW * sizeof(double));
  }
}

void cycle_stage_candidate(mind_cycle *L, size_t o, const double *x0, const double *xs, const double *us, int m) {
  memcpy(L->eval_st.data() + o * 6, x0, 6 * sizeof(double));
  L->eval_ct[o * 2] = 0.0; L->eval_ct[o * 2 + 1] = 0.0;
  memcpy(L->eval_st.data() + (o + 1) * 6, xs, (size_t)m * 6 * sizeof(double));
  memcpy(L->eval_ct.data() + (o + 1) * 2, us, (size_t)m * 2 * sizeof(double));
}

int loop_row(const mind_loop *L, long long n) {
  if (n < L->d.n_steps) return (int)n;
  return L->d.clamp_last ? L->d.n_steps - 1 : -1;
}

void loop_fill_out(const mind_loop *L, mind_loop_out *o) {
  memset(o, 0, sizeof(*o));
  o->planned = L->planned_last ? 1 : 0;
  o->enabled = L->enabled ? 1 : 0;
  o->n_steps = L->n_steps; o->n_plans = L->n_plans; o->episode_steps = L->ep_steps;
  o->sim_time = L->sim_time; o->last_trigger = L->have_trigger ? L->last_trigger : -1.0;
  memcpy(o->state, L->state, sizeof(o->state));
  memcpy(o->ctrl, L->ctrl, sizeof(o->ctrl));
  cycle_fill_plan_out(L, o);
}

void loop_sincos(const mind_loop *L, double x, double *sc) {
  if (L->d.sincos_fn) L->d.sincos_fn(x, sc);
  else { sc[0] = sin(x); sc[1] = cos(x); }
}

void loop_observe(mind_loop *L, int r) {
  const int nt = L->d.n_tracks;
  const double ts = (double)L->timestep[r];
  if (L->obs.empty()) L->slot_of_track[0] = L->add_track(0, 0, L->type_slot[0]);
  const size_t known_before = L->obs.size();
  if (!L->enabled || L->state_recorded) L->obs[0].push_observed(L->ego_obs.data() + (size_t)r * 5, ts);
  else {
    const double *es = L->state;
    double sc[2];
    loop_sincos(L, es[3], sc);
    const double v[5] = {es[0], es[1], es[3], es[2] * sc[1], es[2] * sc[0]};
    L->obs[0].push_observed(v, ts);
  }
  const uint8_t *val = L->exo_valid.data() + (size_t)r * nt;
  for (int i = 1; i < nt; ++i) {
    if (!val[i]) continue;
    int s = L->slot_of_track[i];
// ... 184 lines not shown
    if (t.last()[0] == 0.0) continue;
    L->kept.push_back(t.track); L->kept_keys.push_back(t.key); L->kept_obs.push_back((int32_t)s);
    L->slots.push_back(t.slot);
  }
  const int a = (int)L->kept.size(), T = LOOP_OBS;
  L->raw.assign((size_t)a * T * 6, 0.0);
  for (int i = 0; i < a; ++i) {
    const LoopTrack &t = L->obs[L->kept_obs[i]];
    for (int k = 0; k < t.count; ++k)
      memcpy(L->raw.data() + ((size_t)i * T + (T - t.count + k)) * 6, t.rows[(t.head + k) % LOOP_OBS], 6 * sizeof(double));
  }
  L->f_pos.resize((size_t)a * T * 2); L->f_ang.resize((size_t)a * T); L->f_vel.resize((size_t)a * T * 2);
  L->i_typ.resize((size_t)a * T * 7); L->i_have.resize((size_t)a * T);
  int rc = mind_fill_tracks(L->raw.data(), a, T, L->slots.data(), L->f_pos.data(), L->f_ang.data(), L->f_vel.data(), L->i_typ.data(), L->i_have.data());
  if (rc) return fail(c, rc, "%s: mind_fill_tracks failed", L->who);
  TRL("tracks filled");
  L->f_pad.resize((size_t)a * T); L->f_types.resize((size_t)a * T * 7);
  for (size_t i = 0; i < L->f_pad.size(); ++i) L->f_pad[i] = (float)L->i_have[i];
  for (size_t i = 0; i < L->f_types.size(); ++i) L->f_types[i] = (float)L->i_typ[i];
  mind_aime_plan_in pi;
  memset(&pi, 0, sizeof(pi));
  pi.n_agents = a; pi.n_lanes = d.n_lanes; pi.n_lane_pts = d.n_lane_pts;
  pi.raw_pos = L->f_pos.data(); pi.raw_ang = L->f_ang.data(); pi.raw_vel = L->f_vel.data(); pi.raw_pad = L->f_pad.data();
  pi.types = L->f_types.data();
  pi.target_lane = L->target_lane.data(); pi.target_lane_info = L->target_lane_info.data();
  pi.lane_pts = L->lane_pts.data(); pi.lane_flags = L->lane_flags.data();
  const double cur_vel = L->state[2];
  pi.travel0 = (float)((cur_vel >= (double)d.min_vel ? cur_vel : (double)d.min_vel) * d.time_ahead);
  pi.time_ahead = (float)d.time_ahead; pi.min_vel = d.min_vel; pi.dist_thres = d.dist_thres;
  pi.max_depth = d.max_depth; pi.max_rounds = d.max_rounds; pi.pred_len = d.pred_len; pi.prob_floor = d.prob_floor;
  double *x0 = L->plan_x0;
  x0[0] = L->state[0]; x0[1] = L->state[1]; x0[2] = L->state[2]; x0[3] = L->state[3]; x0[4] = L->ctrl[0]; x0[5] = L->ctrl[1];
  if ((rc = cycle_speculate(L, x0))) return rc;
  if (!L->spec_pending) {
    pi.solve_cfg_warm = &L->cfg_warm; pi.solve_cfg_full = &L->cfg_full;
    pi.solve_x0 = x0; pi.solve_lane = L->solve_lane.data(); pi.solve_n_lane_pts = d.solve_n_lane_pts; pi.solve_target_vel = d.target_vel;
  }
  L->have_plan = false;
  TRL("plan call begins");
  rc = mind_aime_plan(c, &pi, &L->po);
  if (rc) return rc;
  const auto t1 = std::chrono::steady_clock::now();
  TRL("plan returned (solves begun)");
  const int nt = L->po.n_trees;
  if (nt <= 0) return fail(c, MIND_ESTATE, "%s: the plan returned no scenario tree", L->who);
  const int32_t *off = L->po.tree_off;
  const int M = off[nt];
  bool early_done = false;
  const double *xs, *us;
  const mind_ilqr_stats *stw, *stf;
  L->last_agents_plan = a;
  if (L->spec_pending) {
    if ((rc = cycle_solve_speculated(L, x0))) return rc;
    xs = L->sol_xs.data(); us = L->sol_us.data(); stw = L->sol_stw.data(); stf = L->sol_stf.data();
    L->sol_owned = true;
  } else {
    if (!L->po.solves_begun) return fail(c, MIND_ESTATE, "%s: the plan could not begin its contingency solves (%s)", L->who, c->err.c_str());
    if (!c->il_finish || !c->il_finish_owned) return fail(c, MIND_ESTATE, "%s: no plan-begun tree-iLQR call is pending", L->who);
    const mind_ctx::IlEarly E = c->il_early;
    if (c->early_eval && E.done && E.n_trees == nt && E.nodes == (long)M) {
      L->costs.assign(nt, 0.0);
      L->early_seen.assign(nt, 0);
      const void *elane_e = d.eval_lane_is_f32 ? (const void *)L->eval_lane_f32.data() : (const void *)L->eval_lane_f64.data();
      int left = nt;
      const auto te0 = std::chrono::steady_clock::now();
      unsigned spins = 0;
      while (left > 0) {
        bool any = false;
        for (int t = 0; t < nt; ++t) {
          if (L->early_seen[t] || __atomic_load_n((const unsigned *)&E.done[t], __ATOMIC_ACQUIRE) != E.gen) continue;
          const int m = off[t + 1] - off[t];
          L->eval_st.resize((size_t)(m + 1) * 6); L->eval_ct.resize((size_t)(m + 1) * 2);
          cycle_stage_candidate(L, 0, x0, E.xs + (size_t)off[t] * 6, E.us + (size_t)off[t] * 2, m);
          const int32_t cnt1 = m + 1;
          if ((rc = mind_eval_traj_trees(L->eval_st.data(), L->eval_ct.data(), &cnt1, 1, elane_e, d.eval_lane_is_f32, d.eval_n_lane_pts, d.target_vel, &L->costs[t])))
            return fail(c, rc, "%s: mind_eval_traj_trees failed", L->who);
          L->early_seen[t] = 1; --left; any = true;
        }
        if (!any && (++spins & 0x3ffu) == 0u &&
            std::chrono::duration<double>(std::chrono::steady_clock::now() - te0).count() > 0.25) break;
      }
      early_done = left == 0;
    }
    if ((rc = mind_ilqr_finish(c))) return rc;
    if ((size_t)M * 6 != c->pl_sol_xs.size() || (size_t)nt != c->pl_sol_stf.size()) return fail(c, MIND_ESTATE, "%s: the solves' results do not fit the plan", L->who);
    xs = c->pl_sol_xs.data(); us = c->pl_sol_us.data(); stw = c->pl_sol_stw.data(); stf = c->pl_sol_stf.data();
    L->sol_owned = false;
  }
  const auto t2 = std::chrono::steady_clock::now();
  TRL("solves collected");
  if (d.speculative) {
    L->last_shapes.resize(nt);
    for (int t = 0; t < nt; ++t) {
      L->last_shapes[t].parent.assign(L->po.flat_parent + off[t], L->po.flat_parent + off[t + 1]);
      L->last_shapes[t].prob.assign(L->po.flat_prob + off[t], L->po.flat_prob + off[t + 1]);
    }
  }
  L->counts.resize(nt);
  if (early_done) { for (int t = 0; t < nt; ++t) L->counts[t] = off[t + 1] - off[t] + 1; }
  else {
  L->eval_st.resize((size_t)(M + nt) * 6); L->eval_ct.resize((size_t)(M + nt) * 2); L->costs.resize(nt);
  size_t o = 0;
  for (int t = 0; t < nt; ++t) {
    const int m = off[t + 1] - off[t];
    cycle_stage_candidate(L, o, x0, xs + (size_t)off[t] * 6, us + (size_t)off[t] * 2, m);
    L->counts[t] = m + 1;
    o += (size_t)m + 1;
  }
  const void *elane = d.eval_lane_is_f32 ? (const void *)L->eval_lane_f32.data() : (const void *)L->eval_lane_f64.data();
  if ((rc = mind_eval_traj_trees(L->eval_st.data(), L->eval_ct.data(), L->counts.data(), nt, elane, d.eval_lane_is_f32, d.eval_n_lane_pts, d.target_vel, L->costs.data())))
    return fail(c, rc, "%s: mind_eval_traj_trees failed", L->who);
  }
  int best = -1;
  double min_cost = INFINITY;
  for (int t = 0; t < nt; ++t)
    if (L->costs[t] < min_cost) { min_cost = L->costs[t]; best = t; }
  if (best < 0) return fail(c, MIND_ESTATE, "%s: no candidate tree has a finite cost", L->who);
  int first = -1;
  for (int k = off[best]; k < off[best + 1]; ++k)
    if (L->po.flat_parent[k] == -1) { first = k; break; }
  if (first < 0) return fail(c, MIND_ESTATE, "%s: the chosen tree has no root child", L->who);
  L->ctrl[0] = xs[(size_t)first * 6 + 4]; L->ctrl[1] = xs[(size_t)first * 6 + 5];
  L->best = best; L->last_agents = a; L->last_nodes = M; L->have_plan = true; L->plan_gen = c->plan.gen;
  mind_loop_totals &S = L->tot;
  for (int t = 0; t < nt; ++t) {
    const long long m = off[t + 1] - off[t], iw = stw[t].iterations, jf = stf[t].iterations;
    S.iterations += iw + jf; S.node_iterations += m * (iw + jf); S.node_iterations_exo += m * jf * a;
  }
  S.warm_speculated = L->warm_speculated; S.warm_hits = L->warm_hits;
  S.plans += 1; S.expansions += L->po.n_expanded; S.scen_trees += nt; S.rounds += L->po.n_rounds;
  const double N = (double)(a + d.n_lanes + 1);
  S.scene_n2 += (double)L->po.n_expanded * N * N; S.scene_n_a1 += (double)L->po.n_expanded * N * (double)(a + 1);
  if (c->profiling) {
    S.pair_ms += L->po.pair_ms; S.pair_launches += L->po.pair_launches;
    if (c->ilqr_ms > 0.f) {
      S.ilqr_ms += c->ilqr_ms; S.ilqr_launches += 1; S.ilqr_trees += c->ilqr_trees; S.ilqr_workgroups_per_tree = c->ilqr_multi;
      for (int q = 0; q < 9; ++q) S.ilqr_prof[q] += c->il_prof[q];
      S.ilqr_node_steps += c->il_prof[2] * c->il_prof[1];
    }
  }
  const auto t3 = std::chrono::steady_clock::now();
  TRL("evaluated, control chosen");
  L->t_plan_end = t3;
  L->aime_s = std::chrono::duration<double>(t1 - t0).count();
  L->ilqr_s = std::chrono::duration<double>(t2 - t1).count();
  L->total_s = std::chrono::duration<double>(t3 - t0).count();
  S.aime_s += L->aime_s; S.ilqr_s += L->ilqr_s; S.total_s += L->total_s;
  return MIND_OK;
}

int loop_step(mind_loop *L) {
  mind_ctx *c = L->c;
  const mind_loop_desc &d = L->d;
  L->planned_last = false;
  const int r = loop_row(L, L->ep_steps);
  if (r < 0) return fail(c, MIND_EINVAL, "mind_loop: the scene tables end at step %d (episode step %lld)", d.n_steps, L->ep_steps);
  if (L->half_step) return fail(c, MIND_ESTATE, "mind_loop: the plan of the last step failed after its observation update: take the loop over (mind_loop_export) or reset it");
  {
    if (L->sim_time >= d.enable_time && !L->enabled) {
      L->enabled = true;
      memcpy(L->state, L->ego_state.data() + (size_t)r * 4, 4 * sizeof(double));
      L->state_recorded = true; L->state_row = r;
      L->ctrl[0] = 0.0; L->ctrl[1] = 0.0;
    }
    if (!L->have_trigger || (L->sim_time - L->last_trigger) >= d.plan_step) {
      L->have_trigger = true; L->last_trigger = L->sim_time;
      loop_observe(L, r);
      if (L->enabled) {
        const int rc = cycle_plan(L);
        if (rc) {
          L->half_step = true;
          return rc;
        }
        L->n_plans += 1;
        L->planned_last = true;
      }
    }
  }
  if (L->enabled) loop_propagate(L);
  L->sim_time += d.sim_step;
  L->n_steps += 1; L->ep_steps += 1;
  return MIND_OK;
}

}

extern "C" int mind_loop_reset(mind_loop *L);
extern "C" int mind_loop_create(mind_ctx *c, const mind_loop_desc *d, mind_loop **out) {
  if (!c || !d || !out) return MIND_EINVAL;
  if (!c->have_weights) return fail(c, MIND_ESTATE, "weights not loaded");
  if (d->n_tracks <= 0 || d->n_steps <= 0 || !d->ego_state || !d->ego_obs || (d->ego_state_is_f32 && !d->ego_trig32) || !d->exo_obs || !d->exo_valid || !d->timestep || !d->type_slot || !(d->sim_step > 0.0) ||
      !(d->plan_step > 0.0) || !(d->wheelbase > 0.0) || d->n_lanes <= 0 || !d->lane_pts || !d->lane_flags || d->n_lane_pts < 12 || !d->target_lane ||
      !d->target_lane_info || !d->cfg_warm || !d->cfg_full || d->solve_n_lane_pts < 2 || !d->solve_lane || d->eval_n_lane_pts < 2 || !d->eval_lane ||
      d->max_rounds <= 0 || d->max_rounds > 32 || d->pred_len < 2 || d->pred_len > 60)
    return fail(c, MIND_EINVAL, "mind_loop_create: bad argument");
  mind_loop *L = new (std::nothrow) mind_loop();
  if (!L) return fail(c, MIND_ENOMEM, "mind_loop_create: out of memory");
  L->c = c; L->d = *d;
  CycleParams &cp = L->p;
  cycle_params_from(cp, *d);
  cp.n_lanes = d->n_lanes; cp.n_lane_pts = d->n_lane_pts;
  cp.solve_n_lane_pts = d->solve_n_lane_pts; cp.target_vel = d->target_vel;
  cp.eval_n_lane_pts = d->eval_n_lane_pts; cp.eval_lane_is_f32 = d->eval_lane_is_f32;
  const size_t S = (size_t)d->n_steps, nt = (size_t)d->n_tracks;
  L->ego_state.assign(d->ego_state, d->ego_state + S * 4);
  L->ego_obs.assign(d->ego_obs, d->ego_obs + S * 5);
  if (d->ego_trig32) L->ego_trig32.assign(d->ego_trig32, d->ego_trig32 + S * 2);
  L->exo_obs.assign(d->exo_obs, d->exo_obs + S * nt * 5);
  L->exo_valid.assign(d->exo_valid, d->exo_valid + S * nt);
  L->timestep.assign(d->timestep, d->timestep + S);
  L->type_slot.assign(d->type_slot, d->type_slot + nt);
  L->lane_pts.assign(d->lane_pts, d->lane_pts + (size_t)d->n_lanes * 22);
  L->lane_flags.assign(d->lane_flags, d->lane_flags + (size_t)d->n_lanes * 6);
  L->target_lane.assign(d->target_lane, d->target_lane + (size_t)d->n_lane_pts * 2);
  L->target_lane_info.assign(d->target_lane_info, d->target_lane_info + (size_t)d->n_lane_pts * 12);
  L->solve_lane.assign(d->solve_lane, d->solve_lane + (size_t)d->solve_n_lane_pts * 2);
  if (d->eval_lane_is_f32) L->eval_lane_f32.assign((const float *)d->eval_lane, (const float *)d->eval_lane + (size_t)d->eval_n_lane_pts * 2);
  else L->eval_lane_f64.assign((const double *)d->eval_lane, (const double *)d->eval_lane + (size_t)d->eval_n_lane_pts * 2);
  L->cfg_warm = *d->cfg_warm; L->cfg_full = *d->cfg_full;
  L->d.ego_state = nullptr; L->d.ego_obs = nullptr; L->d.ego_trig32 = nullptr; L->d.exo_obs = nullptr; L->d.exo_valid = nullptr; L->d.timestep = nullptr; L->d.type_slot = nullptr; L->d.lane_pts = nullptr;
  L->d.lane_flags = nullptr; L->d.target_lane = nullptr; L->d.target_lane_info = nullptr; L->d.cfg_warm = nullptr; L->d.cfg_full = nullptr;
  L->d.solve_lane = nullptr; L->d.eval_lane = nullptr;
  L->slot_of_track.assign(nt, -1);
  (void)mind_loop_reset(L);
  *out = L;
  return MIND_OK;
}

static void cycle_release(mind_cycle *L) {
  if (L && L->side) {
    (void)mind_ctx_destroy(L->side);
    if (L->side_stream) (void)hipStreamDestroy(L->side_stream);
    L->side = nullptr; L->side_stream = nullptr;
  }
}

extern "C" int mind_loop_destroy(mind_loop *L) {
  cycle_release(L);
  delete L;
  return MIND_OK;
}

extern "C" int mind_loop_reset(mind_loop *L) {
  if (!L) return MIND_EINVAL;
  L->sim_time = 0.0; L->have_trigger = false; L->last_trigger = -1.0; L->enabled = false; L->half_step = false;
  memcpy(L->state, L->ego_state.data(), 4 * sizeof(double));
  L->state_recorded = false; L->tan_valid = false;
  cycle_drop_speculation(L);
  L->ctrl[0] = 0.0; L->ctrl[1] = 0.0;
  L->ep_steps = 0;
  L->obs.clear();
  std::fill(L->slot_of_track.begin(), L->slot_of_track.end(), -1);
  L->planned_last = false;
  return MIND_OK;
}

extern "C" int mind_loop_advance(mind_loop *L, int until_plans, double until_time, long long max_steps, mind_loop_out *out) {
  if (!L || !out || max_steps < 0) return MIND_EINVAL;
  if (L->c->xfn) return fail(L->c, MIND_ESTATE, "mind_loop_advance: the context is sharded (mind_set_exchange): the native loop plans on one GPU");
  int done = 0, rc = MIND_OK;
  bool planned_any = false;
  for (long long s = 0; s < max_steps; ++s) {
    if (until_time >= 0.0 && !(L->sim_time < until_time - 1e-9)) break;
    if ((rc = loop_step(L))) break;
    if (L->planned_last) {
      planned_any = true;
      if (until_plans > 0 && ++done >= until_plans) break;
    }
  }
  L->planned_last = planned_any;
  loop_fill_out(L, out);
  return rc;
}

extern "C" int mind_loop_state(mind_loop *L, mind_loop_out *out) {
  if (!L || !out) return MIND_EINVAL;
  loop_fill_out(L, out);
  return MIND_OK;
}

extern "C" int mind_loop_last_plan(mind_loop *L, mind_aime_plan_out *plan, const double **xs, const double **us, const mind_ilqr_stats **stats_warm,
                                   const mind_ilqr_stats **stats_full, const int32_t **agent_tracks, const float **types, double *x0) {
  if (!L || !plan) return MIND_EINVAL;
  return cycle_last_plan(L, L->kept, plan, xs, us, stats_warm, stats_full, agent_tracks, types, x0);
}

extern "C" int mind_loop_export(mind_loop *L, int cap, int *n, int32_t *track, int32_t *count, double *rows) {
  if (!L || !n) return MIND_EINVAL;
  *n = (int)L->obs.size();
  if (*n > cap || !track || !count || !rows) return MIND_EINVAL;
  cycle_export_rows(L, 0, *n, &LoopTrack::track, track, count, rows);
  return MIND_OK;
}

namespace {

void planner_fill_out(const mind_planner *P, mind_planner_out *o) {
  memset(o, 0, sizeof(*o));
  o->n_plans = P->n_plans;
  if (P->have_plan) memcpy(o->ctrl, P->ctrl, sizeof(o->ctrl));
  cycle_fill_plan_out(P, o);
}

template <class T> bool planner_take(std::vector<T> &dst, const T *src, size_t n) {
  if (dst.size() == n && (n == 0 || memcmp(dst.data(), src, n * sizeof(T)) == 0)) return false;
  dst.assign(src, src + n);
  return true;
}

}

extern "C" int mind_planner_reset(mind_planner *P);
extern "C" int mind_planner_create(mind_ctx *c, const mind_planner_desc *d, mind_planner **out) {
  if (!d || !out) return MIND_EINVAL;
  if (c && !c->have_weights) return fail(c, MIND_ESTATE, "weights not loaded");
  if (!d->cfg_warm || !d->cfg_full || d->max_rounds <= 0 || d->max_rounds > 32 || d->pred_len < 2 || d->pred_len > 60 || d->ego_type_slot < 0 || d->ego_type_slot > 6)
    return fail(c, MIND_EINVAL, "mind_planner_create: bad argument");
  mind_planner *P = new (std::nothrow) mind_planner();
  if (!P) return fail(c, MIND_ENOMEM, "mind_planner_create: out of memory");
  P->c = c; P->who = "mind_planner";
  cycle_params_from(P->p, *d);
  P->cfg_warm = *d->cfg_warm; P->cfg_full = *d->cfg_full;
  P->add_track(0, MIND_PLANNER_EGO_KEY, d->ego_type_slot);
  *out = P;
  return MIND_OK;
}

extern "C" int mind_planner_destroy(mind_planner *P) {
  cycle_release(P);
  delete P;
  return MIND_OK;
}

extern "C" int mind_planner_reset(mind_planner *P) {
  if (!P) return MIND_EINVAL;
  cycle_drop_speculation(P);
  const int ego_slot = P->obs.empty() ? 6 : P->obs[0].slot;
  P->obs.clear();
  P->add_track(0, MIND_PLANNER_EGO_KEY, ego_slot);
  P->slot_of_key.clear();
  P->have_plan = false;
  return MIND_OK;
}

extern "C" int mind_planner_observe(mind_planner *P, int timestep, const double *ego, int n, const long long *track_key, const int32_t *type_slot, const double *rows) {
  if (!P || !ego || n < 0 || (n > 0 && (!track_key || !type_slot || !rows))) return P ? fail(P->c, MIND_EINVAL, "mind_planner_observe: bad argument") : MIND_EINVAL;
  P->frame_keys.assign(track_key, track_key + n);
  std::sort(P->frame_keys.begin(), P->frame_keys.end());
  for (int i = 0; i < n; ++i) {
    if (P->frame_keys[i] == MIND_PLANNER_EGO_KEY) return fail(P->c, MIND_EINVAL, "mind_planner_observe: MIND_PLANNER_EGO_KEY names the ego's own track");
    if (i > 0 && P->frame_keys[i] == P->frame_keys[i - 1]) return fail(P->c, MIND_EINVAL, "mind_planner_observe: track key %lld twice in one frame", P->frame_keys[i]);
    if (type_slot[i] < 0 || type_slot[i] > 6) return fail(P->c, MIND_EINVAL, "mind_planner_observe: type slot %d of track %d", (int)type_slot[i], i);
  }
  const size_t known_before = P->obs.size();
  P->obs[0].push_observed(ego, (double)timestep);
  P->frame_seen.assign(known_before, 0);
  for (int i = 0; i < n; ++i) {
    int s;
    auto it = P->slot_of_key.find(track_key[i]);
    if (it == P->slot_of_key.end()) {
      s = P->add_track((int)P->obs.size(), track_key[i], type_slot[i]);
      P->slot_of_key.emplace(track_key[i], s);
    } else {
      s = it->second;
      P->frame_seen[s] = 1;
    }
    P->obs[s].push_observed(rows + (size_t)i * 5, (double)timestep);
  }
  cycle_repeat_unseen(P, known_before, [&](size_t s, const LoopTrack &) { return P->frame_seen[s] != 0; });
  return MIND_OK;
}

extern "C" int mind_planner_set_lanes(mind_planner *P, int n_lanes, const double *lane_pts, const int32_t *lane_flags) {
  if (!P) return MIND_EINVAL;
  if (!P->c) return MIND_ESTATE;
  if (n_lanes <= 0 || !lane_pts || !lane_flags) return fail(P->c, MIND_EINVAL, "mind_planner_set_lanes: bad argument");
  bool ch = planner_take(P->lane_pts, lane_pts, (size_t)n_lanes * 22);
  ch = planner_take(P->lane_flags, lane_flags, (size_t)n_lanes * 6) || ch;
  P->p.n_lanes = n_lanes; P->have_lanes = true; P->n_uploads += ch;
  return MIND_OK;
}

extern "C" int mind_planner_set_target_lane(mind_planner *P, int n, const float *lane, const float *info) {
  if (!P) return MIND_EINVAL;
  if (!P->c) return MIND_ESTATE;
  if (!lane || !info) return fail(P->c, MIND_EINVAL, "mind_planner_set_target_lane: bad argument");
  if (n < 12) return fail(P->c, MIND_EINVAL, "mind_planner_set_target_lane: a target lane of %d points (the plan needs 12)", n);
  bool ch = planner_take(P->target_lane, lane, (size_t)n * 2);
  ch = planner_take(P->target_lane_info, info, (size_t)n * 12) || ch;
  P->p.n_lane_pts = n; P->have_target = true; P->n_uploads += ch;
  return MIND_OK;
}

extern "C" int mind_planner_set_solve_lane(mind_planner *P, int n, const double *lane, double target_vel) {
  if (!P) return MIND_EINVAL;
  if (!P->c) return MIND_ESTATE;
  if (n < 2 || !lane) return fail(P->c, MIND_EINVAL, "mind_planner_set_solve_lane: bad argument");
  const bool ch = planner_take(P->solve_lane, lane, (size_t)n * 2);
  P->p.solve_n_lane_pts = n; P->p.target_vel = target_vel; P->have_solve = true; P->n_uploads += ch;
  return MIND_OK;
}

extern "C" int mind_planner_set_eval_lane(mind_planner *P, int n, const void *lane, int is_f32) {
  if (!P) return MIND_EINVAL;
  if (!P->c) return MIND_ESTATE;
  if (n < 2 || !lane) return fail(P->c, MIND_EINVAL, "mind_planner_set_eval_lane: bad argument");
  bool ch;
  if (is_f32) { ch = planner_take(P->eval_lane_f32, (const float *)lane, (size_t)n * 2); P->eval_lane_f64.clear(); }
  else { ch = planner_take(P->eval_lane_f64, (const double *)lane, (size_t)n * 2); P->eval_lane_f32.clear(); }
  P->p.eval_n_lane_pts = n; P->p.eval_lane_is_f32 = is_f32 ? 1 : 0; P->have_eval = true; P->n_uploads += ch;
  return MIND_OK;
}

extern "C" int mind_planner_plan(mind_planner *P, const double *state, const double *ctrl, mind_planner_out *out) {
  if (!P || !state || !ctrl || !out) return MIND_EINVAL;
  if (!P->c) return MIND_ESTATE;
  mind_ctx *c = P->c;
  if (c->xfn) return fail(c, MIND_ESTATE, "mind_planner_plan: the context is sharded (mind_set_exchange): the native cycle plans on one GPU");
  if (P->obs[0].count == 0) return fail(c, MIND_ESTATE, "mind_planner_plan: no observation yet (mind_planner_observe)");
  if (!P->have_lanes) return fail(c, MIND_ESTATE, "mind_planner_plan: the lane tables are not set (mind_planner_set_lanes)");
  if (!P->have_target || !P->have_solve || !P->have_eval)
    return fail(c, MIND_ESTATE, "mind_planner_plan: the target lane is not set (mind_planner_set_target_lane / _set_solve_lane / _set_eval_lane)");
  memcpy(P->state, state, 4 * sizeof(double));
  memcpy(P->ctrl, ctrl, 2 * sizeof(double));
  const int rc = cycle_plan(P);
  if (rc == MIND_OK) P->n_plans += 1;
  planner_fill_out(P, out);
  return rc;
}

extern "C" int mind_planner_last_plan(mind_planner *P, mind_aime_plan_out *plan, const double **xs, const double **us, const mind_ilqr_stats **stats_warm,
                                      const mind_ilqr_stats **stats_full, const long long **agent_keys, const float **types, double *x0) {
  if (!P || !plan) return MIND_EINVAL;
  if (!P->c) return MIND_ESTATE;
  return cycle_last_plan(P, P->kept_keys, plan, xs, us, stats_warm, stats_full, agent_keys, types, x0);
}

extern "C" int mind_planner_export(mind_planner *P, int cap, int *n, long long *key, int32_t *count, double *rows) {
  if (!P || !n) return MIND_EINVAL;
  const int first = P->obs[0].count ? 0 : 1;
  *n = (int)P->obs.size() - first;
  if (*n > cap || (*n > 0 && (!key || !count || !rows))) return MIND_EINVAL;
  cycle_export_rows(P, first, *n, &LoopTrack::key, key, count, rows);
  return MIND_OK;
}
```

### mind_amd/csrc/mind_hip.hip

```cpp
#include <hip/hip_runtime.h>

#include <cmath>
#include <cstdarg>
#include <cstdio>
#include <cstdlib>
#include <algorithm>
#include <cstring>
#include <map>
#include <string>
#include <thread>
#include <atomic>
#include <functional>
#include <vector>

#include "../../include/mind_hip.h"
#include "encdec_kernels.hip"
#include "fusion_kernels.hip"
#include "pair_bf16_kernels.hip"
#include "pair_tile_kernels.hip"
#include "pair_tile6_kernels.hip"
#include "token_mfma_kernels.hip"
#include "actor_mfma_kernels.hip"
#include "actor_lw_kernels.hip"
#include "token_lw_kernels.hip"
#include "actor_f32_kernels.hip"
#include "dec_mfma_kernels.hip"
#include "dec_curve_kernels.hip"
#include "ilqr_kernels.hip"
#include "ilqr_score_kernels.hip"
#include "ilqr_policy_kernels.hip"
#include "audit_kernels.hip"
#include "forecast_kernels.hip"
#include "road_kernels.hip"
#include "pair_jobs.h"
#include "pred_choice.h"
#include "ilqr_choice.h"
#include "aime_book.h"
#include "weight_pack.h"
#include "aime_kernels.hip"

namespace {

struct DevBuf {
  void *p = nullptr;
  size_t cap = 0;
};

}

struct TableSet {
  std::vector<int> key;
  DevBuf meta, jobs, jobs5, rows;
  std::vector<int> actor_row, cls_row, scene_n;
  long long edge_pairs = 0, edge_pairs_t = 0, stamp = 0;
  int ntok = 0, slot = 0, njobs = 0, njobs5 = 0;
  double pairs_full = 0, pairs_l5 = 0;
};
#define MIND_TABLE_SETS 8

struct mind_ctx {
  int device = 0;
  hipStream_t stream = nullptr;
  bool own_stream = false;
  hipStream_t side = nullptr;
  hipEvent_t ev_side = nullptr, ev_main = nullptr, ev_stage = nullptr, ev_tgt = nullptr, ev_cls = nullptr;
  std::vector<char> aime_stage;
  bool aime_stage_busy = false;
  std::string err;
  float *wdev = nullptr;
  bool have_weights = false;
  WeightTables W = {};
  PredTuning pt;
  int dec_basis = MIND_BASIS_BEZIER;
  DevBuf curve_tab;
  std::vector<double> curve_tau;
  int curve_tab_basis = -1;
  DevBuf tok_lw_arena;
  std::vector<TlLaunch> tok_lw_plan;
  int last_tok_lw = 0, last_tok_launches = 0, last_tok_chunks = 0;
  float tok_ms = 0.f, tok_stage_ms[TL_NSTAGE + 1] = {};
  std::vector<hipEvent_t> ev_tok;
  std::vector<int> ev_tok_tag;
  TableSet tabs[MIND_TABLE_SETS];
  long long tab_clock = 0;
  long long n_table_hits = 0;
  IlqrTuning it;
  int upload_kernel_max = 1 << 20;
  bool dec_mirror = true;
  bool glue_fused = true;
  bool dec_poll = true;
  unsigned dec_gen = 0;
  DevBuf pl_cnt;
  bool root_head = true, round_head = true;
  std::function<int(hipStream_t)> enc_pre, enc_post;
  bool early_eval = true;
  int tab_host_max = 4096;
  bool tab_small = true;
  std::vector<IlTables> il_tab;
  struct IlImage { std::vector<double> hD; std::vector<float> hF; std::vector<int> hI; } il_img;
  struct IlEarly { const double *xs = nullptr, *us = nullptr; volatile unsigned *done = nullptr; unsigned gen = 0; int n_trees = 0; long nodes = 0; } il_early;
  unsigned il_gen = 0;
  long long il_spec_req = 0, il_spec_hit = 0;
  DevBuf actor_lw_arena;
  std::vector<LwLaunch> actor_lw_plan;
  int last_actor_lw = 0, last_actor_launches = 0, last_actor_chunks = 0;
  float actor_ms = 0.f;
  hipEvent_t ev_act0 = nullptr, ev_act1 = nullptr;
  int pair_prec = 3;
  int plan_chunk_mb = 96 * 1024;
  std::vector<int> last_scene_n;
  bool last_edge_tiled = false, last_edge_bf16 = false;
  DevBuf edge, x, ST, QK, part, tokpos, meta, jobs, actor_feat, lane_feat, tgt_feat, cmode, tgt_emb,
      rows, rpe_ptrs;
  DevBuf ilqr_dev, aime_dev, rebase_dev2[2], dec_h2;
  DevBuf audit_dev;
  DevBuf forecast_dev;
  DevBuf road_dev;
  DevBuf pl_root, pl_in[2], pl_lf, pl_lrep, pl_pred, pl_small, pl_tab[2], pl_win[2];
  std::vector<DevBuf> pl_world;
  void *pl_pin[8] = {nullptr, nullptr, nullptr, nullptr, nullptr, nullptr, nullptr, nullptr};
  size_t pl_pin_cap[8] = {0, 0, 0, 0, 0, 0, 0, 0};
  hipEvent_t ev_pl = nullptr, ev_tab = nullptr, ev_root = nullptr;
  DevBuf il_field;
  void *il_field_pin = nullptr;
  size_t il_field_pin_cap = 0;
  hipEvent_t ev_field = nullptr;
  bool il_field_valid = false;
  double il_field_key[5] = {0, 0, 0, 0, 0};
  std::vector<double> il_field_lane;
  int xr = 0, xw = 1;
  mind_exchange_fn xfn = nullptr;
  void *xuser = nullptr;
  bool xforce = false;
  DevBuf x_send, x_recv, x_seg;
  long long x_collectives = 0, x_bytes = 0;
  hipStream_t pl_copy = nullptr;
  bool pl_tab_side = false;
  std::vector<double> pl_sol_xs, pl_sol_us;
  std::vector<mind_ilqr_stats> pl_sol_stw, pl_sol_stf;
  std::thread pa_thread;
  std::atomic<int> pa_state{0};
  mind_aime_plan_in pa_in;
  mind_aime_plan_out pa_out;
  int pa_rc = 0;
  struct Plan {
    AimeBook book;
    int agents = 0;
    long long gen = 0;
    const float *rows_p = nullptr, *fmean_p = nullptr, *fcov_p = nullptr;
    const float *dev_fmean = nullptr, *dev_fcov = nullptr;
  } plan;
  DevBuf pl_flat;
  DevBuf dec_xbuf, dec_bars;
  unsigned *dec_abort = nullptr;
  int rb_cur = 0, rb_gen = 0;
  size_t rb_S = 0, rb_a = 0;
  bool profiling = false;
  hipEvent_t ev_il0 = nullptr, ev_il1 = nullptr;
  float ilqr_ms = 0.f;
  int ilqr_multi = 0, ilqr_trees = 0;
  std::function<int()> il_finish;
  bool il_finish_owned = false;
  hipEvent_t ev_rows = nullptr;
  std::vector<const double *> il_trace_dev;
  std::vector<int> il_trace_its;
  int il_trace_cap = 0, il_trace_phases = 0;
  double il_prof[9] = {0, 0, 0, 0, 0, 0, 0, 0, 0};
  long long n_ilqr_fallbacks = 0;
  int n_pair_launch = 0;
  float pair_ms = 0.f;
  double pairs_done = 0.0;
  std::vector<hipEvent_t> ev;
  bool ev_defer = false;
  std::vector<hipEvent_t> ev_pool;
  size_t ev_pool_used = 0;
  std::vector<size_t> ev_pending;
  int n_cu = 256;
  int debug_layers = 6;
  int last_ntok = 0;
  size_t il_dbg[6] = {0, 0, 0, 0, 0, 0};
  long long last_edge_pairs = 0;
  int last_slots = 0, last_A = 0, last_B = 0;
};

static int fail(mind_ctx *c, int code, const char *fmt, ...) {
  char buf[512];
  va_list ap;
  va_start(ap, fmt);
  vsnprintf(buf, sizeof(buf), fmt, ap);
  va_end(ap);
  if (c) c->err = buf;
  return code;
}

#define HIPCHK(c, call)                                                                        \
  do {                                                                                         \
    hipError_t e_ = (call);                                                                    \
    if (e_ != hipSuccess)                                                                      \
      return fail(c, MIND_EHIP, "%s failed: %s (%s:%d)", #call, hipGetErrorString(e_), __FILE__, __LINE__); \
  } while (0)

static int ensure(mind_ctx *c, DevBuf &b, size_t bytes) {
  if (bytes <= b.cap) return MIND_OK;
  if (b.p) (void)hipFree(b.p);
  b.p = nullptr;
  b.cap = 0;
  size_t want = bytes < ((size_t)64 << 20) ? std::max<size_t>(2 * bytes, (size_t)1 << 20) : bytes + bytes / 4 + 4096;
  hipError_t e = hipMalloc(&b.p, want);
  if (e != hipSuccess) {
    e = hipMalloc(&b.p, bytes);
    want = bytes;
    if (e != hipSuccess) return fail(c, MIND_ENOMEM, "hipMalloc(%zu) failed: %s", bytes, hipGetErrorString(e));
  }
  b.cap = want;
  return MIND_OK;
}

static int ensure_exact(mind_ctx *c, DevBuf &b, size_t bytes, const char *what) {
  if (bytes <= b.cap) return MIND_OK;
  HIPCHK(c, hipStreamSynchronize(c->stream));
  if (b.p) (void)hipFree(b.p);
  b.p = nullptr;
  b.cap = 0;
  if (hipMalloc(&b.p, bytes) != hipSuccess) return fail(c, MIND_ENOMEM, "hipMalloc(%zu) for %s failed", bytes, what);
  b.cap = bytes;
  return MIND_OK;
}

extern "C" int mind_ctx_create(int device, void *stream, mind_ctx **out) {
  if (!out) return MIND_EINVAL;
  *out = nullptr;
  int n = 0;
  if (hipGetDeviceCount(&n) != hipSuccess || n <= 0) return MIND_EHIP;
  if (device < 0 || device >= n) return MIND_EINVAL;
  mind_ctx *c = new mind_ctx();
  c->device = device;
  if (hipSetDevice(device) != hipSuccess) { delete c; return MIND_EHIP; }
  c->stream = (hipStream_t)stream;
  if (hipStreamCreateWithFlags(&c->side, hipStreamNonBlocking) != hipSuccess) c->side = nullptr;
  if (c->side && hipEventCreateWithFlags(&c->ev_side, hipEventDisableTiming) != hipSuccess) { (void)hipStreamDestroy(c->side); c->side = nullptr; }
  if (c->side && hipEventCreateWithFlags(&c->ev_main, hipEventDisableTiming) != hipSuccess) { (void)hipStreamDestroy(c->side); c->side = nullptr; }
  if (c->side && hipEventCreateWithFlags(&c->ev_tgt, hipEventDisableTiming) != hipSuccess) { (void)hipStreamDestroy(c->side); c->side = nullptr; }
  if (hipEventCreateWithFlags(&c->ev_stage, hipEventDisableTiming) != hipSuccess) { *out = nullptr; delete c; return MIND_EHIP; }
  hipDeviceProp_t prop;
  if (hipGetDeviceProperties(&prop, device) == hipSuccess) c->n_cu = prop.multiProcessorCount;
  (void)hipFuncSetAttribute((const void *)k_pair<0>, hipFuncAttributeMaxDynamicSharedMemorySize, (int)mind_pair_lds_bytes());
  (void)hipFuncSetAttribute((const void *)k_pair<1>, hipFuncAttributeMaxDynamicSharedMemorySize, (int)mind_pair_lds_bytes());
  (void)hipFuncSetAttribute((const void *)k_pair_bf<0, 3>, hipFuncAttributeMaxDynamicSharedMemorySize, (int)mind_pair_bf_lds_bytes());
  (void)hipFuncSetAttribute((const void *)k_pair_bf<1, 3>, hipFuncAttributeMaxDynamicSharedMemorySize, (int)mind_pair_bf_lds_bytes());
  (void)hipFuncSetAttribute((const void *)k_pair_bf<0, 1>, hipFuncAttributeMaxDynamicSharedMemorySize, (int)mind_pair_bf_lds_bytes());
  (void)hipFuncSetAttribute((const void *)k_pair_bf<1, 1>, hipFuncAttributeMaxDynamicSharedMemorySize, (int)mind_pair_bf_lds_bytes());
  (void)hipFuncSetAttribute((const void *)k_pair_t<0, 3>, hipFuncAttributeMaxDynamicSharedMemorySize, (int)mind_pair_bf_lds_bytes());
  (void)hipFuncSetAttribute((const void *)k_pair_t<1, 3>, hipFuncAttributeMaxDynamicSharedMemorySize, (int)mind_pair_bf_lds_bytes());
  (void)hipFuncSetAttribute((const void *)k_pair_t<0, 1>, hipFuncAttributeMaxDynamicSharedMemorySize, (int)mind_pair_bf_lds_bytes());
  (void)hipFuncSetAttribute((const void *)k_pair_t<1, 1>, hipFuncAttributeMaxDynamicSharedMemorySize, (int)mind_pair_bf_lds_bytes());
  (void)hipFuncSetAttribute((const void *)k_pair_t6<0>, hipFuncAttributeMaxDynamicSharedMemorySize, (int)mind_pair_bf_lds_bytes());
  (void)hipFuncSetAttribute((const void *)k_pair_t6<1>, hipFuncAttributeMaxDynamicSharedMemorySize, (int)mind_pair_bf_lds_bytes());
  if (const char *te = getenv("MIND_PAIR_TILE")) c->pt.pair_tile = !(te[0] == '0');
  if (const char *xe = getenv("MIND_XCD_ORDER")) c->pt.xcd_order = !(xe[0] == '0');

  if (const char *pe = getenv("MIND_PAIR_PREC")) {
    const std::string v = pe;
    if (v == "f32" || v == "0") c->pair_prec = 0;
    else if (v == "bf16x3" || v == "1") c->pair_prec = 1;
    else if (v == "bf16" || v == "2") c->pair_prec = 2;
    else if (v == "bf16x6" || v == "3") c->pair_prec = 3;
  }
  (void)hipFuncSetAttribute((const void *)k_actor_net, hipFuncAttributeMaxDynamicSharedMemorySize, (int)mind_actor_lds_bytes());
  (void)hipFuncSetAttribute((const void *)k_actor_mfma<3>, hipFuncAttributeMaxDynamicSharedMemorySize, (int)mind_actor_mfma_lds_bytes());
  (void)hipFuncSetAttribute((const void *)k_actor_mfma<6>, hipFuncAttributeMaxDynamicSharedMemorySize, (int)mind_actor_mfma_lds_bytes());
  (void)hipFuncSetAttribute((const void *)k_dec_actor_mfma<1>, hipFuncAttributeMaxDynamicSharedMemorySize, (int)mind_dec_actor_mfma_lds_bytes());
  (void)hipFuncSetAttribute((const void *)k_dec_actor_mfma<3>, hipFuncAttributeMaxDynamicSharedMemorySize, (int)mind_dec_actor_mfma_lds_bytes());
  (void)hipFuncSetAttribute((const void *)k_dec_actor_mfma<6>, hipFuncAttributeMaxDynamicSharedMemorySize, (int)mind_dec_actor_mfma_lds_bytes());
  if (const char *se = getenv("MIND_ACTOR_SPLIT")) c->pt.actor_np = atoi(se) == 3 ? 3 : 6;
  (void)hipFuncSetAttribute((const void *)k_actor_mfma<1>, hipFuncAttributeMaxDynamicSharedMemorySize, (int)mind_actor_mfma_lds_bytes());
  if (const char *me = getenv("MIND_ENC_MFMA")) c->pt.enc_mfma = !(me[0] == '0');
  if (const char *me = getenv("MIND_ACTOR_F32")) c->pt.actor_f32 = !(me[0] == '0');
  if (const char *me = getenv("MIND_ACTOR_F32_MIN")) c->pt.actor_f32_min = atoi(me);
  if (const char *me = getenv("MIND_ACTOR_LW_MIN")) c->pt.actor_lw_min = atoi(me);
  lw_set_attributes();
  (void)hipFuncSetAttribute((const void *)k_actor_f32<1>, hipFuncAttributeMaxDynamicSharedMemorySize, (int)mind_actor_f32_lds_bytes(1));
  (void)hipFuncSetAttribute((const void *)k_actor_f32<2>, hipFuncAttributeMaxDynamicSharedMemorySize, (int)mind_actor_f32_lds_bytes(2));
  if (const char *de = getenv("MIND_DEC_MFMA_MIN")) c->pt.dec_mfma_min = atoi(de);
  if (const char *oe = getenv("MIND_DEC_OVERLAP")) c->pt.dec_overlap = !(oe[0] == '0');
  (void)hipFuncSetAttribute((const void *)k_ilqr<true, 0>, hipFuncAttributeMaxDynamicSharedMemorySize, (int)il_lds_bytes(0));
  (void)hipFuncSetAttribute((const void *)k_ilqr<false, 1>, hipFuncAttributeMaxDynamicSharedMemorySize, (int)il_lds_bytes(0));
  (void)hipFuncSetAttribute((const void *)k_ilqr<false, 0>, hipFuncAttributeMaxDynamicSharedMemorySize, (int)il_lds_bytes(0));
  (void)hipFuncSetAttribute((const void *)k_ilqr<false, 2>, hipFuncAttributeMaxDynamicSharedMemorySize, (int)il_lds_bytes(0));
  if (const char *te = getenv("MIND_TOK_MFMA")) c->pt.tok_mfma = !(te[0] == '0');
  if (const char *te = getenv("MIND_TOK_SMALL_MAX")) c->pt.tok_small_max = atoi(te);
  if (const char *te = getenv("MIND_TOK_MERGE")) c->pt.tok_merge = !(te[0] == '0');
  if (const char *te = getenv("MIND_DEC_MW")) c->pt.dec_mw = !(te[0] == '0');
  if (const char *te = getenv("MIND_DEC_CLS_SIDE")) c->pt.dec_cls_side = !(te[0] == '0');
  if (const char *te = getenv("MIND_TOK_BF_MIN_N")) c->pt.tok_bf_min_n = atoi(te);
  if (const char *te = getenv("MIND_TOK_LW_MIN_N")) c->pt.tok_lw_min_n = atoi(te);
  if (const char *te = getenv("MIND_TOK_LW_MIN")) c->pt.tok_lw_min = atoi(te);
  if (const char *te = getenv("MIND_TGT_SIDE")) c->pt.tgt_side = !(te[0] == '0');
  if (const char *te = getenv("MIND_PL_TAB_SIDE")) c->pl_tab_side = !(te[0] == '0');
  (void)hipFuncSetAttribute((const void *)k_token_mfma<0>, hipFuncAttributeMaxDynamicSharedMemorySize, (int)mind_token_mfma_lds_bytes());
  (void)hipFuncSetAttribute((const void *)k_token_mfma<1>, hipFuncAttributeMaxDynamicSharedMemorySize, (int)mind_token_mfma_lds_bytes());
  if (const char *ce = getenv("MIND_PLAN_CHUNK_MB")) { const long v = atol(ce); if (v > 0) c->plan_chunk_mb = v; }
  if (const char *we = getenv("MIND_TAB_SMALL")) c->tab_small = atoi(we) != 0;
  if (const char *we = getenv("MIND_TAB_HOST_MAX")) c->tab_host_max = std::max(0, atoi(we));
  if (const char *we = getenv("MIND_EARLY_EVAL")) c->early_eval = atoi(we) != 0;
  if (const char *we = getenv("MIND_GLUE_FUSED")) c->glue_fused = atoi(we) != 0;
  if (const char *we = getenv("MIND_DEC_MIRROR")) c->dec_mirror = atoi(we) != 0;
  if (const char *we = getenv("MIND_DEC_POLL")) c->dec_poll = atoi(we) != 0;
  if (const char *we = getenv("MIND_ROOT_HEAD")) c->root_head = atoi(we) != 0;
  if (const char *we = getenv("MIND_ROUND_HEAD")) c->round_head = atoi(we) != 0;
  if (const char *we = getenv("MIND_UPLOAD_KERNEL_MAX")) c->upload_kernel_max = std::max(0, atoi(we));
  const char *const il_env[][2] = {{"MIND_ILQR_CHUNK", "ilqr_chunk"}, {"MIND_ILQR_WGS", "ilqr_wgs"}, {"MIND_ILQR_SPEC_DERIV", "ilqr_spec_deriv"},
                                   {"MIND_ILQR_HOST_OUT_MAX", "ilqr_host_out_max"}, {"MIND_ILQR_SLOTS", "ilqr_slots"}};
  for (const auto &e : il_env)
    if (const char *we = getenv(e[0])) (void)ilqr_tuning_set(c->it, e[1], atoi(we));
  (void)hipFuncSetAttribute((const void *)k_dec_scene, hipFuncAttributeMaxDynamicSharedMemorySize, (int)mind_dec_scene_lds_bytes());
  (void)hipFuncSetAttribute((const void *)k_dec_scene_mw, hipFuncAttributeMaxDynamicSharedMemorySize, (int)mind_dec_scene_lds_bytes());
  (void)hipFuncSetAttribute((const void *)k_dec_scene_c, hipFuncAttributeMaxDynamicSharedMemorySize, (int)mind_dec_scene_lds_bytes());
  (void)hipFuncSetAttribute((const void *)k_dec_cls, hipFuncAttributeMaxDynamicSharedMemorySize, (int)mind_dec_scene_lds_bytes());
  (void)hipFuncSetAttribute((const void *)k_dec_tgt, hipFuncAttributeMaxDynamicSharedMemorySize, (int)mind_dec_scene_lds_bytes());
  (void)hipFuncSetAttribute((const void *)k_dec_actor<0>, hipFuncAttributeMaxDynamicSharedMemorySize, (int)mind_dec_actor_lds_bytes());
  (void)hipFuncSetAttribute((const void *)k_dec_actor<1>, hipFuncAttributeMaxDynamicSharedMemorySize, (int)mind_dec_actor_lds_bytes());
  (void)hipFuncSetAttribute((const void *)k_dec_actor<2>, hipFuncAttributeMaxDynamicSharedMemorySize, (int)mind_dec_actor_lds_bytes());
  (void)hipFuncSetAttribute((const void *)k_dec_actor<2, 1>, hipFuncAttributeMaxDynamicSharedMemorySize, (int)mind_dec_actor_lds_bytes());
  (void)hipFuncSetAttribute((const void *)k_dec_actor<2, 2>, hipFuncAttributeMaxDynamicSharedMemorySize, (int)mind_dec_actor_lds_bytes());
  if (const char *te = getenv("MIND_DEC_HEAD_RA")) (void)pred_tuning_set(c->pt, "dec_head_ra", atoi(te));
  *out = c;
  return MIND_OK;
}

extern "C" int mind_ctx_destroy(mind_ctx *c) {
  if (!c) return MIND_EINVAL;
  if (c->pa_thread.joinable()) c->pa_thread.join();
  (void)hipSetDevice(c->device);
  (void)hipStreamSynchronize(c->stream);
  DevBuf *bufs[] = {&c->edge, &c->x, &c->ST, &c->QK, &c->part, &c->tokpos, &c->meta, &c->jobs, &c->actor_feat,
                    &c->lane_feat, &c->tgt_feat, &c->cmode, &c->tgt_emb, &c->rows, &c->rpe_ptrs, &c->ilqr_dev, &c->aime_dev, &c->rebase_dev2[0], &c->rebase_dev2[1], &c->dec_h2,
                    &c->curve_tab, &c->audit_dev, &c->forecast_dev, &c->road_dev};
  for (DevBuf *b : bufs)
    if (b->p) (void)hipFree(b->p);
  for (TableSet &t : c->tabs)
    for (DevBuf *b : {&t.meta, &t.jobs, &t.jobs5, &t.rows})
      if (b->p) (void)hipFree(b->p);
  if (c->wdev) (void)hipFree(c->wdev);
  for (DevBuf *b : {&c->dec_xbuf, &c->dec_bars})
    if (b->p) (void)hipFree(b->p);
  if (c->dec_abort) (void)hipHostFree(c->dec_abort);
  for (DevBuf *b : {&c->pl_root, &c->pl_in[0], &c->pl_in[1], &c->pl_lf, &c->pl_lrep, &c->pl_pred, &c->pl_small, &c->pl_tab[0], &c->pl_tab[1], &c->pl_win[0],
                    &c->pl_win[1], &c->pl_flat, &c->x_send, &c->x_recv, &c->x_seg, &c->pl_cnt})
    if (b->p) (void)hipFree(b->p);
  for (DevBuf &b : c->pl_world)
    if (b.p) (void)hipFree(b.p);
  for (void *q : c->pl_pin)
    if (q) (void)hipHostFree(q);
  if (c->ev_pl) (void)hipEventDestroy(c->ev_pl);
  if (c->ev_root) (void)hipEventDestroy(c->ev_root);
  if (c->ev_field) (void)hipEventDestroy(c->ev_field);
  if (c->il_field.p) (void)hipFree(c->il_field.p);
  if (c->il_field_pin) (void)hipHostFree(c->il_field_pin);
  if (c->ev_tab) (void)hipEventDestroy(c->ev_tab);
  if (c->ev_rows) (void)hipEventDestroy(c->ev_rows);
  if (c->pl_copy) (void)hipStreamDestroy(c->pl_copy);
  for (hipEvent_t e : c->ev) (void)hipEventDestroy(e);
  for (hipEvent_t e : c->ev_pool) (void)hipEventDestroy(e);
  if (c->ev_side) (void)hipEventDestroy(c->ev_side);
  if (c->ev_main) (void)hipEventDestroy(c->ev_main);
  if (c->ev_tgt) (void)hipEventDestroy(c->ev_tgt);
  if (c->ev_stage) (void)hipEventDestroy(c->ev_stage);
  if (c->ev_cls) (void)hipEventDestroy(c->ev_cls);
  if (c->actor_lw_arena.p) (void)hipFree(c->actor_lw_arena.p);
  if (c->tok_lw_arena.p) (void)hipFree(c->tok_lw_arena.p);
  for (hipEvent_t e : c->ev_tok) (void)hipEventDestroy(e);
  if (c->ev_act0) (void)hipEventDestroy(c->ev_act0);
  if (c->ev_act1) (void)hipEventDestroy(c->ev_act1);
  if (c->ev_il0) (void)hipEventDestroy(c->ev_il0);
  if (c->ev_il1) (void)hipEventDestroy(c->ev_il1);
  if (c->side) { (void)hipStreamSynchronize(c->side); (void)hipStreamDestroy(c->side); }
  if (c->own_stream) (void)hipStreamDestroy(c->stream);
  delete c;
  return MIND_OK;
}

extern "C" const char *mind_last_error_string(mind_ctx *c) { return c ? c->err.c_str() : "null context"; }

extern "C" int mind_ctx_synchronize(mind_ctx *c) {
  if (!c) return MIND_EINVAL;
  HIPCHK(c, hipStreamSynchronize(c->stream));
  return MIND_OK;
}

extern "C" int mind_set_tuning(mind_ctx *c, const char *name, int value) {
  if (!c || !name) return MIND_EINVAL;
  const std::string n = name;
  if (pred_tuning_set(c->pt, name, value)) return MIND_OK;
  if (ilqr_tuning_set(c->it, name, value)) return MIND_OK;
  if (n == "plan_chunk_mb") c->plan_chunk_mb = value < 1 ? 1 : value;
  else if (n == "pl_tab_side") c->pl_tab_side = value != 0;
  else if (n == "tab_small") c->tab_small = value != 0;
  else if (n == "tab_host_max") c->tab_host_max = value < 0 ? 0 : value;
  else if (n == "early_eval") c->early_eval = value != 0;
  else if (n == "glue_fused") c->glue_fused = value != 0;
  else if (n == "dec_mirror") c->dec_mirror = value != 0;
  else if (n == "dec_poll") c->dec_poll = value != 0;
  else if (n == "root_head") c->root_head = value != 0;
  else if (n == "round_head") c->round_head = value != 0;
  else if (n == "upload_kernel_max") c->upload_kernel_max = value < 0 ? 0 : value;
  else return fail(c, MIND_EINVAL, "mind_set_tuning: unknown knob '%s'", name);
  return MIND_OK;
}

extern "C" int mind_set_exchange(mind_ctx *c, int rank, int world, mind_exchange_fn fn, void *user, int force) {
  if (!c) return MIND_EINVAL;
  if (fn && (world < 1 || rank < 0 || rank >= world)) return fail(c, MIND_EINVAL, "mind_set_exchange: rank %d of %d", rank, world);
  c->xfn = fn; c->xuser = user;
  c->xr = fn ? rank : 0; c->xw = fn ? world : 1; c->xforce = fn && force != 0;
  return MIND_OK;
}

extern "C" int mind_last_exchange_stats(mind_ctx *c, long long *collectives, long long *bytes) {
  if (!c) return MIND_EINVAL;
  if (collectives) *collectives = c->x_collectives;
  if (bytes) *bytes = c->x_bytes;
  return MIND_OK;
}

extern "C" int mind_set_pair_precision(mind_ctx *c, int mode) {
  if (!c || mode < 0 || mode > 3) return MIND_EINVAL;
  c->pair_prec = mode;
  return MIND_OK;
}

extern "C" int mind_get_pair_precision(mind_ctx *c) { return c ? c->pair_prec : MIND_EINVAL; }

extern "C" int mind_debug_pack_bfrag(const float *w, int row_stride, uint32_t *out) {
  if (!w || !out || row_stride < 128) return MIND_EINVAL;
  std::vector<float> v(w, w + (size_t)127 * row_stride + 128);
  v.resize((size_t)128 * row_stride, 0.f);
  const std::vector<float> t = pack_bfrag(v, row_stride);
  memcpy(out, t.data(), 16384 * sizeof(uint32_t));
  return MIND_OK;
}

extern "C" int mind_set_profiling(mind_ctx *c, int enable) {
  if (!c) return MIND_EINVAL;
  c->profiling = enable != 0;
  return MIND_OK;
}

extern "C" int mind_last_ilqr_stats(mind_ctx *c, float *kernel_ms, int *n_trees, int *workgroups_per_tree) {
  if (!c) return MIND_EINVAL;
  if (kernel_ms) *kernel_ms = c->ilqr_ms;
  if (n_trees) *n_trees = c->ilqr_trees;
  if (workgroups_per_tree) *workgroups_per_tree = c->ilqr_multi;
  return MIND_OK;
}

extern "C" int mind_last_ilqr_trace(mind_ctx *c, int tree, int phase, double *out, int cap_rows, int *n_rows) {
  if (!c || !n_rows || (cap_rows > 0 && !out)) return MIND_EINVAL;
  if (tree < 0 || tree >= (int)c->il_trace_dev.size() || phase < 0 || phase >= c->il_trace_phases || !c->il_trace_dev[tree])
    return fail(c, MIND_ESTATE, "mind_last_ilqr_trace: no trace for tree %d phase %d (the last tree-iLQR call had %d trees, %d phases)", tree, phase,
                (int)c->il_trace_dev.size(), c->il_trace_phases);
  const int rows = std::min(c->il_trace_its[2 * tree + phase], c->il_trace_cap);
  *n_rows = rows;
  const int take = std::min(rows, cap_rows);
  if (take > 0) {
    HIPCHK(c, hipMemcpyAsync(out, c->il_trace_dev[tree] + (size_t)phase * c->il_trace_cap * IL_TRACE_W, (size_t)take * IL_TRACE_W * sizeof(double),
                             hipMemcpyDeviceToHost, c->stream));
    HIPCHK(c, hipStreamSynchronize(c->stream));
  }
  return MIND_OK;
}

extern "C" int mind_last_ilqr_profile(mind_ctx *c, double *out9) {
  if (!c || !out9) return MIND_EINVAL;
  memcpy(out9, c->il_prof, sizeof(c->il_prof));
  return MIND_OK;
}

static int mind_pair_events_resolve(mind_ctx *c, float *total_ms) {
  float sum = 0.f;
  for (size_t base : c->ev_pending)
    for (int L = 0; L < c->debug_layers; ++L) {
      float ms = 0.f;
      HIPCHK(c, hipEventElapsedTime(&ms, c->ev_pool[base + 2 * L], c->ev_pool[base + 2 * L + 1]));
      sum += ms;
    }
  c->ev_pending.clear();
  c->ev_pool_used = 0;
  *total_ms = sum;
  return MIND_OK;
}

extern "C" int mind_last_fusion_stats(mind_ctx *c, int *n_launches, float *total_ms, double *pairs) {
  if (!c) return MIND_EINVAL;
  if (n_launches) *n_launches = c->n_pair_launch;
  if (total_ms) *total_ms = c->pair_ms;
  if (pairs) *pairs = c->pairs_done;
  return MIND_OK;
}

extern "C" int mind_last_actor_stats(mind_ctx *c, int *layerwise, int *n_launches, int *n_chunks, float *total_ms) {
  if (!c) return MIND_EINVAL;
  if (layerwise) *layerwise = c->last_actor_lw;
  if (n_launches) *n_launches = c->last_actor_launches;
  if (n_chunks) *n_chunks = c->last_actor_chunks;
  if (total_ms) *total_ms = c->actor_ms;
  return MIND_OK;
}

extern "C" int mind_last_token_stats(mind_ctx *c, int *layerwise, int *n_launches, int *n_chunks, float *total_ms) {
  if (!c) return MIND_EINVAL;
  if (layerwise) *layerwise = c->last_tok_lw;
  if (n_launches) *n_launches = c->last_tok_launches;
  if (n_chunks) *n_chunks = c->last_tok_chunks;
  if (total_ms) *total_ms = c->tok_ms;
  return MIND_OK;
}

extern "C" int mind_last_token_stage_ms(mind_ctx *c, float *out_ms, int cap) {
  if (!c || cap < 0 || (cap > 0 && !out_ms)) return MIND_EINVAL;
  for (int i = 0; i < cap && i <= TL_NSTAGE; ++i) out_ms[i] = c->tok_stage_ms[i];
  return TL_NSTAGE + 1;
}

extern "C" int mind_debug_token_lw_plan(int n_tokens, int mode, int chunk, long long *out_launches, int cap, long long *out_info) {
  if (n_tokens <= 0 || chunk < 0 || !tl_mode_ok(mode) || (cap > 0 && !out_launches) || cap < 0) return MIND_EINVAL;
  if (chunk == 0) chunk = TL_CHUNK;
  std::vector<TlLaunch> plan;
  tl_build_plan(n_tokens, mode, chunk, TL_NCU_PLAN, plan);
  for (size_t i = 0; i < plan.size() && (int)i < cap; ++i) {
    const TlLaunch &L = plan[i];
    long long *o = out_launches + 8 * i;
    o[0] = L.stage; o[1] = L.gx; o[2] = L.gy; o[3] = L.block; o[4] = L.lds; o[5] = L.t0; o[6] = L.n; o[7] = (L.n + TM_TOK - 1) / TM_TOK;
  }
  if (out_info) {
    out_info[0] = chunk; out_info[1] = (long long)tl_arena_bytes(chunk); out_info[2] = (long long)plan.size();
    out_info[3] = (n_tokens + chunk - 1) / chunk;
  }
  return (int)plan.size();
}

extern "C" int mind_debug_actor_lw_plan(int n_actors, int np, int chunk, long long *out_launches, int cap, long long *out_info) {
  if (n_actors <= 0 || chunk < 0 || (np != 1 && np != 3 && np != 6) || (cap > 0 && !out_launches) || cap < 0) return MIND_EINVAL;
  if (chunk == 0) chunk = LW_CHUNK;
  std::vector<LwLaunch> plan;
  lw_build_plan(n_actors, chunk, plan);
  LwStage S[LW_NSTAGE];
  lw_stages(S);
  const int nparts = np == 6 ? 3 : (np == 3 ? 2 : 1);
  for (size_t i = 0; i < plan.size() && (int)i < cap; ++i) {
    const LwLaunch &L = plan[i];
    long long *o = out_launches + 16 * i;
// ... 625 lines not shown
```

Measured before the change: 1824.

## Defer tree-iLQR stream synchronize to a lazy event drain

When the early-eval path has already consumed the solves' results, finishing the tree-iLQR no longer blocks on hipStreamSynchronize. It records a completion event and marks the work as owed. Later entry points that reuse buffers or need timing (pin reallocation, next solve, field upload, loop advance end, destroy, stats) drain the event first. This removes a host stall per planning cycle and lets host work overlap the kernel tail, at the cost of more synchronisation bookkeeping and a risk of races if some buffer-reuse path misses a drain.

```diff
diff --git a/include/mind_hip.h b/include/mind_hip.h
--- a/include/mind_hip.h
+++ b/include/mind_hip.h
@@ -79,6 +79,7 @@
 int mind_last_token_stage_ms(mind_ctx *ctx, float *out_ms, int cap);
 int mind_last_ilqr_stats(mind_ctx *ctx, float *kernel_ms, int *n_trees, int *workgroups_per_tree);
 int mind_last_ilqr_profile(mind_ctx *ctx, double *out9);
+int mind_solve_lazy_stats(mind_ctx *ctx, long long *out4);
 int mind_last_ilqr_trace(mind_ctx *ctx, int tree, int phase, double *out, int cap_rows, int *n_rows);
 int mind_set_profiling(mind_ctx *ctx, int enable);
 
diff --git a/mind_amd/_lib.py b/mind_amd/_lib.py
--- a/mind_amd/_lib.py
+++ b/mind_amd/_lib.py
@@ -214,7 +214,7 @@
 EXPORTS = ["mind_ctx_create", "mind_ctx_destroy", "mind_last_error_string", "mind_ctx_synchronize",
            "mind_weights_load", "mind_predict_batch", "mind_last_fusion_stats", "mind_last_actor_stats", "mind_debug_actor_lw_plan", "mind_last_token_stats", "mind_last_token_stage_ms", "mind_debug_token_lw_plan", "mind_set_profiling",
            "mind_ilqr_solve_trees", "mind_ilqr_contingency", "mind_ilqr_solve_fields", "mind_cost_eval", "mind_ilqr_score_trees", "mind_ilqr_gains", "mind_ilqr_policy_rollouts", "mind_lane_dist_field", "mind_aime_world", "mind_aime_rebase", "mind_debug_aime_decide", "mind_debug_set_layers",
-           "mind_debug_read", "mind_set_pair_precision", "mind_get_pair_precision", "mind_debug_pack_bfrag", "mind_debug_pack_conv_frag", "mind_debug_pack", "mind_debug_weight_image", "mind_debug_weight_bind", "mind_debug_pair_schedule", "mind_debug_predict_choice", "mind_debug_ilqr_plan", "mind_debug_aime_book", "mind_set_tuning", "mind_last_ilqr_stats", "mind_aime_plan", "mind_last_ilqr_profile", "mind_eval_traj_trees", "mind_last_ilqr_trace", "mind_ilqr_contingency_begin", "mind_ilqr_finish", "mind_fill_tracks", "mind_ilqr_contingency_begin_plan", "mind_debug_trig", "mind_aime_plan_begin", "mind_aime_plan_poll", "mind_aime_plan_finish", "mind_ctx_busy", "mind_ilqr_finish_plan",
+           "mind_debug_read", "mind_set_pair_precision", "mind_get_pair_precision", "mind_debug_pack_bfrag", "mind_debug_pack_conv_frag", "mind_debug_pack", "mind_debug_weight_image", "mind_debug_weight_bind", "mind_debug_pair_schedule", "mind_debug_predict_choice", "mind_debug_ilqr_plan", "mind_debug_aime_book", "mind_set_tuning", "mind_last_ilqr_stats", "mind_aime_plan", "mind_last_ilqr_profile", "mind_solve_lazy_stats", "mind_eval_traj_trees", "mind_last_ilqr_trace", "mind_ilqr_contingency_begin", "mind_ilqr_finish", "mind_fill_tracks", "mind_ilqr_contingency_begin_plan", "mind_debug_trig", "mind_aime_plan_begin", "mind_aime_plan_poll", "mind_aime_plan_finish", "mind_ctx_busy", "mind_ilqr_finish_plan",
            "mind_set_exchange", "mind_last_exchange_stats", "mind_debug_wait_word",
            "mind_predict_batch_aux", "mind_set_decoder_basis", "mind_get_decoder_basis", "mind_curve_eval", "mind_debug_curve_basis",
            "mind_audit_plan", "mind_audit_episode", "mind_debug_box_clearance",
@@ -304,6 +304,7 @@
     lib.mind_set_tuning.argtypes = [C.c_void_p, C.c_char_p, C.c_int]
     lib.mind_last_ilqr_stats.argtypes = [C.c_void_p, C.POINTER(C.c_float), C.POINTER(C.c_int), C.POINTER(C.c_int)]
     lib.mind_last_ilqr_profile.argtypes = [C.c_void_p, C.POINTER(C.c_double)]
+    lib.mind_solve_lazy_stats.argtypes = [C.c_void_p, C.POINTER(C.c_longlong)]
     lib.mind_last_ilqr_trace.argtypes = [C.c_void_p, C.c_int, C.c_int, C.POINTER(C.c_double), C.c_int, C.POINTER(C.c_int)]
     lib.mind_eval_traj_trees.argtypes = [C.POINTER(C.c_double), C.POINTER(C.c_double), C.POINTER(C.c_int32), C.c_int, C.c_void_p, C.c_int, C.c_int,
                                          C.c_double, C.POINTER(C.c_double)]
diff --git a/mind_amd/csrc/aime_plan.hip b/mind_amd/csrc/aime_plan.hip
--- a/mind_amd/csrc/aime_plan.hip
+++ b/mind_amd/csrc/aime_plan.hip
@@ -3,6 +3,8 @@
 
 int pl_pin(mind_ctx *c, int which, size_t bytes) {
   if (bytes <= c->pl_pin_cap[which]) return MIND_OK;
+  const int rc = il_drain(c);
+  if (rc) return rc;
   if (c->pl_pin[which]) (void)hipHostFree(c->pl_pin[which]);
   c->pl_pin[which] = nullptr; c->pl_pin_cap[which] = 0;
   const size_t want = bytes < ((size_t)64 << 20) ? std::max<size_t>(2 * bytes, (size_t)1 << 20) : bytes + bytes / 2 + 4096;
@@ -597,6 +599,7 @@
   const size_t Mtot = (size_t)book.tree_off.back(), n_rows = (size_t)book.n_rows, n_flat = Mtot * a * 3, n_res = n_rows + n_flat;
   want_solves = solves_asked() && !book.tree_top.empty();
   int rc;
+  if ((rc = il_drain(c))) return rc;
   c->plan.agents = a;
   c->plan.rows_p = c->plan.fmean_p = c->plan.fcov_p = nullptr;
   c->plan.dev_fmean = c->plan.dev_fcov = nullptr;
diff --git a/mind_amd/csrc/ilqr_host.hip b/mind_amd/csrc/ilqr_host.hip
--- a/mind_amd/csrc/ilqr_host.hip
+++ b/mind_amd/csrc/ilqr_host.hip
@@ -56,6 +56,7 @@
   if (W < 3 || H < 3 || n_lane_pts < 2 || !(cfg->grid_res > 0)) return MIND_OK;
   const size_t nin = (size_t)W + H + 2 * (size_t)n_lane_pts, nd = nin + (size_t)W * H;
   int rc;
+  if ((rc = il_drain(c))) return rc;
   if ((rc = ensure(c, c->il_field, nd * sizeof(double)))) return rc;
   if (c->il_field_pin_cap < nin * sizeof(double)) {
     if (c->il_field_pin) (void)hipHostFree(c->il_field_pin);
@@ -404,6 +405,7 @@
   mind_ilqr_stats *stats, *stats2;
   struct Tree { int M, nl, nseg, nsl, maxls, a; const double *trace; };
   std::vector<Tree> tree;
+  hipEvent_t ev_done = nullptr;
 };
 
 static void il_launch_kernel(const IlPending &P, int form) {
@@ -423,12 +425,17 @@
   return MIND_OK;
 }
 
-static int il_finish_run(mind_ctx *c, const IlPending &P) {
+static int il_finish_run(mind_ctx *c, const IlPending &P, bool lazy) {
   static const bool trace = getenv("MIND_ILQR_TRACE") != nullptr;
   const int n_trees = P.n_trees, n_phases = P.n_phases;
   int rc;
-  HIPCHK(c, hipStreamSynchronize(P.st));
-  if (c->profiling) HIPCHK(c, hipEventElapsedTime(&c->ilqr_ms, c->ev_il0, c->ev_il1));
+  if (lazy && P.ev_done && P.ch.early && P.ch.form != 1) {
+    c->il_owed.owed = true; c->il_owed.ev = P.ev_done; c->il_owed.prof = P.ev_done == c->ev_il1; c->il_owed.ms_sink = nullptr;
+    c->n_il_lazy++;
+  } else {
+    HIPCHK(c, hipStreamSynchronize(P.st));
+    if (c->profiling) HIPCHK(c, hipEventElapsedTime(&c->ilqr_ms, c->ev_il0, c->ev_il1));
+  }
   if (P.ch.form == 1 && *P.h_abort) {
     c->n_ilqr_fallbacks++;
     HIPCHK(c, hipMemcpyAsync(P.base, P.up, P.o_work, hipMemcpyHostToDevice, P.st));
@@ -598,6 +605,14 @@
   il_launch_kernel(P, ch.form);
   HIPCHK(c, hipGetLastError());
   if (c->profiling) HIPCHK(c, hipEventRecord(c->ev_il1, st));
+  if (c->solve_lazy && ch.early && q.begin_only) {
+    if (c->profiling) P.ev_done = c->ev_il1;
+    else {
+      if (!c->ev_il_done) HIPCHK(c, hipEventCreateWithFlags(&c->ev_il_done, hipEventDisableTiming));
+      HIPCHK(c, hipEventRecord(c->ev_il_done, st));
+      P.ev_done = c->ev_il_done;
+    }
+  }
   int rc;
   if ((rc = il_read_back(c, P))) return rc;
   if (ch.form == 1) HIPCHK(c, hipMemcpyAsync(R.h_abort, P.dBars + 4 * (size_t)n_trees, sizeof(unsigned), hipMemcpyDeviceToHost, st));
@@ -609,6 +624,7 @@
   int rc;
   if ((rc = il_check(c, q, R))) return rc;
   HIPCHK(c, hipSetDevice(c->device));
+  if ((rc = il_drain(c))) return rc;
   hipStream_t st = c->stream;
   IlStamp stamp;
   il_grid(R);
@@ -632,8 +648,8 @@
   IlPending P;
   if ((rc = il_launch(c, R, st, P)) || other) return rc;
   stamp("kernel launched");
-  if (!q.begin_only) return il_finish_run(c, P);
-  c->il_finish = [c, P = std::move(P)]() { return il_finish_run(c, P); };
+  if (!q.begin_only) return il_finish_run(c, P, false);
+  c->il_finish = [c, P = std::move(P)](bool lazy) { return il_finish_run(c, P, lazy); };
   return MIND_OK;
 }
 
@@ -679,14 +695,18 @@
   return il_solve(c, q);
 }
 
+static int il_finish_pending(mind_ctx *c, bool lazy) {
+  std::function<int(bool)> fin = std::move(c->il_finish);
+  c->il_finish = nullptr;
+  c->il_finish_owned = false;
+  c->il_early = mind_ctx::IlEarly();
+  return fin(lazy);
+}
+
 extern "C" int mind_ilqr_finish(mind_ctx *c) {
   if (!c) return MIND_EINVAL;
   if (!c->il_finish) return fail(c, MIND_ESTATE, "mind_ilqr_finish: no tree-iLQR call was begun on this context");
-  std::function<int()> fin = std::move(c->il_finish);
-  c->il_finish = nullptr;
-  c->il_finish_owned = false;
-  c->il_early = mind_ctx::IlEarly();
-  return fin();
+  return il_finish_pending(c, false);
 }
 
 extern "C" int mind_ilqr_contingency(mind_ctx *c, const mind_ilqr_cfg *cfg_warm, const mind_ilqr_cfg *cfg_full,
diff --git a/mind_amd/csrc/loop.hip b/mind_amd/csrc/loop.hip
--- a/mind_amd/csrc/loop.hip
+++ b/mind_amd/csrc/loop.hip
@@ -126,6 +126,7 @@
 }
 
 void cycle_drop_speculation(mind_cycle *L) {
+  if (L->c) (void)il_drain(L->c);
   if (L->spec_pending && L->side) { (void)mind_ilqr_finish(L->side); L->spec_pending = false; }
 }
 
@@ -476,7 +477,7 @@
       }
       early_done = left == 0;
     }
-    if ((rc = mind_ilqr_finish(c))) return rc;
+    if ((rc = il_finish_pending(c, early_done && c->solve_lazy))) return rc;
     if ((size_t)M * 6 != c->pl_sol_xs.size() || (size_t)nt != c->pl_sol_stf.size()) return fail(c, MIND_ESTATE, "%s: the solves' results do not fit the plan", L->who);
     xs = c->pl_sol_xs.data(); us = c->pl_sol_us.data(); stw = c->pl_sol_stw.data(); stf = c->pl_sol_stf.data();
     L->sol_owned = false;
@@ -527,8 +528,11 @@
   S.scene_n2 += (double)L->po.n_expanded * N * N; S.scene_n_a1 += (double)L->po.n_expanded * N * (double)(a + 1);
   if (c->profiling) {
     S.pair_ms += L->po.pair_ms; S.pair_launches += L->po.pair_launches;
-    if (c->ilqr_ms > 0.f) {
-      S.ilqr_ms += c->ilqr_ms; S.ilqr_launches += 1; S.ilqr_trees += c->ilqr_trees; S.ilqr_workgroups_per_tree = c->ilqr_multi;
+    const bool owed = c->il_owed.owed && c->il_owed.prof;
+    if (owed) c->il_owed.ms_sink = &S.ilqr_ms;
+    if (owed || c->ilqr_ms > 0.f) {
+      if (!owed) S.ilqr_ms += c->ilqr_ms;
+      S.ilqr_launches += 1; S.ilqr_trees += c->ilqr_trees; S.ilqr_workgroups_per_tree = c->ilqr_multi;
       for (int q = 0; q < 9; ++q) S.ilqr_prof[q] += c->il_prof[q];
       S.ilqr_node_steps += c->il_prof[2] * c->il_prof[1];
     }
@@ -622,6 +626,7 @@
 }
 
 static void cycle_release(mind_cycle *L) {
+  if (L && L->c) (void)il_drain(L->c);
   if (L && L->side) {
     (void)mind_ctx_destroy(L->side);
     if (L->side_stream) (void)hipStreamDestroy(L->side_stream);
@@ -663,8 +668,9 @@
     }
   }
   L->planned_last = planned_any;
+  const int rc_d = il_drain(L->c);
   loop_fill_out(L, out);
-  return rc;
+  return rc ? rc : rc_d;
 }
 
 extern "C" int mind_loop_state(mind_loop *L, mind_loop_out *out) {
@@ -681,6 +687,7 @@
 
 extern "C" int mind_loop_export(mind_loop *L, int cap, int *n, int32_t *track, int32_t *count, double *rows) {
   if (!L || !n) return MIND_EINVAL;
+  (void)il_drain(L->c);
   *n = (int)L->obs.size();
   if (*n > cap || !track || !count || !rows) return MIND_EINVAL;
   cycle_export_rows(L, 0, *n, &LoopTrack::track, track, count, rows);
@@ -817,7 +824,9 @@
     return fail(c, MIND_ESTATE, "mind_planner_plan: the target lane is not set (mind_planner_set_target_lane / _set_solve_lane / _set_eval_lane)");
   memcpy(P->state, state, 4 * sizeof(double));
   memcpy(P->ctrl, ctrl, 2 * sizeof(double));
-  const int rc = cycle_plan(P);
+  int rc = cycle_plan(P);
+  const int rc_d = il_drain(c);
+  if (rc == MIND_OK) rc = rc_d;
   if (rc == MIND_OK) P->n_plans += 1;
   planner_fill_out(P, out);
   return rc;
diff --git a/mind_amd/csrc/mind_hip.hip b/mind_amd/csrc/mind_hip.hip
--- a/mind_amd/csrc/mind_hip.hip
+++ b/mind_amd/csrc/mind_hip.hip
@@ -94,6 +94,14 @@
   bool root_head = true, round_head = true;
   std::function<int(hipStream_t)> enc_pre, enc_post;
   bool early_eval = true;
+  bool solve_lazy = true;
+  struct IlDrain {
+    bool owed = false, prof = false;
+    hipEvent_t ev = nullptr;
+    double *ms_sink = nullptr;
+  } il_owed;
+  hipEvent_t ev_il_done = nullptr;
+  long long n_il_lazy = 0, n_il_drain_ready = 0, n_il_drain_wait = 0;
   int tab_host_max = 4096;
   bool tab_small = true;
   std::vector<IlTables> il_tab;
@@ -159,7 +167,7 @@
   hipEvent_t ev_il0 = nullptr, ev_il1 = nullptr;
   float ilqr_ms = 0.f;
   int ilqr_multi = 0, ilqr_trees = 0;
-  std::function<int()> il_finish;
+  std::function<int(bool)> il_finish;
   bool il_finish_owned = false;
   hipEvent_t ev_rows = nullptr;
   std::vector<const double *> il_trace_dev;
@@ -213,6 +221,21 @@
     if (e != hipSuccess) return fail(c, MIND_ENOMEM, "hipMalloc(%zu) failed: %s", bytes, hipGetErrorString(e));
   }
   b.cap = want;
+  return MIND_OK;
+}
+
+static int il_drain(mind_ctx *c) {
+  if (!c->il_owed.owed) return MIND_OK;
+  const mind_ctx::IlDrain d = c->il_owed;
+  c->il_owed = mind_ctx::IlDrain();
+  hipError_t e = hipEventQuery(d.ev);
+  if (e == hipSuccess) c->n_il_drain_ready++;
+  else if (e == hipErrorNotReady) { c->n_il_drain_wait++; e = hipEventSynchronize(d.ev); }
+  if (e != hipSuccess) return fail(c, MIND_EHIP, "tree-iLQR drain: %s", hipGetErrorString(e));
+  if (d.prof) {
+    HIPCHK(c, hipEventElapsedTime(&c->ilqr_ms, c->ev_il0, c->ev_il1));
+    if (d.ms_sink) *d.ms_sink += c->ilqr_ms;
+  }
   return MIND_OK;
 }
 
@@ -303,6 +326,7 @@
   if (const char *we = getenv("MIND_TAB_SMALL")) c->tab_small = atoi(we) != 0;
   if (const char *we = getenv("MIND_TAB_HOST_MAX")) c->tab_host_max = std::max(0, atoi(we));
   if (const char *we = getenv("MIND_EARLY_EVAL")) c->early_eval = atoi(we) != 0;
+  if (const char *we = getenv("MIND_SOLVE_LAZY")) c->solve_lazy = atoi(we) != 0;
   if (const char *we = getenv("MIND_GLUE_FUSED")) c->glue_fused = atoi(we) != 0;
   if (const char *we = getenv("MIND_DEC_MIRROR")) c->dec_mirror = atoi(we) != 0;
   if (const char *we = getenv("MIND_DEC_POLL")) c->dec_poll = atoi(we) != 0;
@@ -332,6 +356,7 @@
   if (!c) return MIND_EINVAL;
   if (c->pa_thread.joinable()) c->pa_thread.join();
   (void)hipSetDevice(c->device);
+  (void)il_drain(c);
   (void)hipStreamSynchronize(c->stream);
   DevBuf *bufs[] = {&c->edge, &c->x, &c->ST, &c->QK, &c->part, &c->tokpos, &c->meta, &c->jobs, &c->actor_feat,
                     &c->lane_feat, &c->tgt_feat, &c->cmode, &c->tgt_emb, &c->rows, &c->rpe_ptrs, &c->ilqr_dev, &c->aime_dev, &c->rebase_dev2[0], &c->rebase_dev2[1], &c->dec_h2,
@@ -374,6 +399,7 @@
   if (c->ev_act1) (void)hipEventDestroy(c->ev_act1);
   if (c->ev_il0) (void)hipEventDestroy(c->ev_il0);
   if (c->ev_il1) (void)hipEventDestroy(c->ev_il1);
+  if (c->ev_il_done) (void)hipEventDestroy(c->ev_il_done);
   if (c->side) { (void)hipStreamSynchronize(c->side); (void)hipStreamDestroy(c->side); }
   if (c->own_stream) (void)hipStreamDestroy(c->stream);
   delete c;
@@ -384,6 +410,8 @@
 
 extern "C" int mind_ctx_synchronize(mind_ctx *c) {
   if (!c) return MIND_EINVAL;
+  int rc;
+  if ((rc = il_drain(c))) return rc;
   HIPCHK(c, hipStreamSynchronize(c->stream));
   return MIND_OK;
 }
@@ -398,6 +426,7 @@
   else if (n == "tab_small") c->tab_small = value != 0;
   else if (n == "tab_host_max") c->tab_host_max = value < 0 ? 0 : value;
   else if (n == "early_eval") c->early_eval = value != 0;
+  else if (n == "solve_lazy") c->solve_lazy = value != 0;
   else if (n == "glue_fused") c->glue_fused = value != 0;
   else if (n == "dec_mirror") c->dec_mirror = value != 0;
   else if (n == "dec_poll") c->dec_poll = value != 0;
@@ -448,6 +477,8 @@
 
 extern "C" int mind_last_ilqr_stats(mind_ctx *c, float *kernel_ms, int *n_trees, int *workgroups_per_tree) {
   if (!c) return MIND_EINVAL;
+  int rc;
+  if ((rc = il_drain(c))) return rc;
   if (kernel_ms) *kernel_ms = c->ilqr_ms;
   if (n_trees) *n_trees = c->ilqr_trees;
   if (workgroups_per_tree) *workgroups_per_tree = c->ilqr_multi;
@@ -467,6 +498,12 @@
                              hipMemcpyDeviceToHost, c->stream));
     HIPCHK(c, hipStreamSynchronize(c->stream));
   }
+  return MIND_OK;
+}
+
+extern "C" int mind_solve_lazy_stats(mind_ctx *c, long long *out4) {
+  if (!c || !out4) return MIND_EINVAL;
+  out4[0] = c->n_il_lazy; out4[1] = c->n_il_drain_ready; out4[2] = c->n_il_drain_wait; out4[3] = c->il_owed.owed ? 1 : 0;
   return MIND_OK;
 }
 
```

New measurement: 1835, median of 6. Within noise of the previous version (+0.6%).
